# MingXiangL/SPE

Measured on AMD Instinct MI355X. Metric: images/sec (whole node) at 3x800x1333 bs=2/GPU, higher is better.
Workload: dtype bf16/fp16 operands, fp32 accumulate; 1 GPU; TSCAM_cait_S24 (C=384, depth 24, 8 heads) + 0-layer encoder + 6-layer conditional-DETR decoder x2 stages, 100 queries, COCO heads (91), 2x3x800x1333 per GPU (N=4150 tokens), fwd + SetCriterion + SetCriterionRefine + bwd + grad all-reduce + clip + AdamW; global_batch=2, parallelism=dp1

## Files before the change

### include/spe_hip.h

```cpp
#ifndef SPE_HIP_H
#define SPE_HIP_H
#include <stddef.h>
#include <stdint.h>

#ifdef __cplusplus
extern "C" {
#endif

typedef struct ihipStream_t* spe_stream_t;

int spe_abi_version(void);

int spe_set_reduce_workspace(void* ws, size_t bytes, spe_stream_t stream);
int spe_reduce_defer_ranges(const void* const* ptrs, const size_t* bytes, int n);
int spe_reduce_defer_arena(void* arena, size_t bytes);
int spe_reduce_flush(spe_stream_t stream);
int spe_reduce_pending(void);

int spe_gemm_f32(const float* A, const float* B, float* C, const float* bias, float* C2,
                 int M, int N, int K, long lda, long ldb, long ldc, int transA, int transB,
                 int batch0, int batch1, long sA0, long sA1, long sB0, long sB1, long sC0, long sC1,
                 float alpha, int act, int splitk, int precision, spe_stream_t stream);

int spe_gemm_ex(const void* A, int a_bf16, const float* B, float* C, const float* bias, float* C2,
                int M, int N, int K, long lda, long ldb, long ldc, int transA, int transB,
                int batch0, int batch1, long sA0, long sA1, long sB0, long sB1, long sC0, long sC1,
                float alpha, int act, int splitk, int precision, spe_stream_t stream);

int spe_gemm_tile(int M, int N, int nbatch);

int spe_layernorm_fwd(const float* x, const float* gamma, const float* beta, float* y, float* mean,
                      float* rstd, long R, int C, float eps, void* y16, void* y16lo, spe_stream_t stream);
int spe_layernorm_fwd_h(const float* x, const float* gamma, const float* beta, float* y, float* mean,
                        float* rstd, long R, int C, float eps, void* y16, void* yh16, spe_stream_t stream);
int spe_layernorm_bwd(const float* dy, const float* x, const float* gamma, const float* mean,
                      const float* rstd, float* dx, float* dgamma, float* dbeta, long R, int C,
                      const float* add, spe_stream_t stream);
int spe_layernorm_bwd_ls(const float* dy, const float* x, const float* gamma, const float* mean, const float* rstd, float* dx,
                         float* dgamma, float* dbeta, long R, int C, const float* add, const float* ls_y, const float* ls_gamma,
                         void* ls_dy16, float* ls_db, float* ls_dg, spe_stream_t stream);

int spe_cvt_f16(const float* x, long ldx, int R, int C, void* out, long ldo, spe_stream_t stream);
int spe_gemm_bf16nt(const void* A16, const void* B16, const void* A16lo, const void* B16lo, float* C, const float* bias,
                    float* C2, int M, int N, int K, long lda, long ldb, long ldc, float alpha, int act, int splitk,
                    spe_stream_t stream);
int spe_linear_small_fwd(const float* x, long ldx, const void* W16, const void* W16lo, const float* bias, float* y, float* pre,
                         void* x16_out, int R, int N, int K, long ldc, int act, spe_stream_t stream);
int spe_linear_small_bwd(const float* dy, const float* aux, int act, const void* x16, const void* WT16, float* dx, float* dW,
                         float* db, int R, int N, int K, spe_stream_t stream);
int spe_linear_small_group_fwd(const float* x, long ldx, const void* const* W16, const void* const* W16lo, const float* const* bias,
                               const float* const* add, float* const* y, void* x16_out, int R, int nblk, int N, int K, spe_stream_t stream);
int spe_linear_small_group_bwd(const float* const* dy, const void* x16, const void* const* WT16, float* dx, float* const* dW,
                               float* const* db, int R, int nblk, int N, int K, spe_stream_t stream);
int spe_gemm_bf16tn(const void* A16, const void* B16, float* C, int M, int N, int R, long lda, long ldb, long ldc,
                    float alpha, int splitk, spe_stream_t stream);
int spe_gemm_bf16tn_plan(int M, int N, int R, long lda, long ldb, int splitk, int* v);
int spe_gemm_bf16nt_ex(const void* A16, const void* B16, const void* A16lo, const void* B16lo, float* C, const float* bias,
                       float* C2, void* out16, void* out16lo, long ld16, void* out16T, long ld16t, float* colsum, const float* aux,
                       const float* res, const float* rgamma, int M, int N, int K, long lda, long ldb, long ldc, float alpha, int act,
                       int half_flags, spe_stream_t stream);
int spe_gemm_bf16nt_exd(const void* A16, const void* B16, const void* A16lo, const void* B16lo, float* C, const float* bias,
                        float* C2, void* out16, void* out16lo, long ld16, void* out16T, long ld16t, float* colsum, const float* aux,
                        const float* res, const float* rgamma, int M, int N, int K, long lda, long ldb, long ldc, float alpha, int act,
                        int half_flags, float p_drop, uint64_t seed, uint64_t offset, const float* sample_scale, long rows_per_sample,
                        spe_stream_t stream);
int spe_gemm_bf16nt_plan(int M, int N, int K, int split, int ex, int f16_operands, int f16_second, int splitk, int has_out16t,
                         long ld16t, int* plan);
int spe_cvt_bf16(const float* x, long ldx, int R, int C, void* out, void* out_lo, long ldo, void* outT, long ldt, float* colsum,
                 const float* aux, int act, spe_stream_t stream);
int spe_cvt_bf16_h(const float* x, long ldx, int R, int C, void* out, void* out_h, long ldo, void* outT, long ldt, spe_stream_t stream);
int spe_cvt_bf16_multi(const void* jobs_dev, int njobs, int total_tiles, spe_stream_t stream);

int spe_softmax_fwd(const float* S, const unsigned char* mask, float* P, float* Pd, int B, int H, int Nq,
                    int Nk, long ld, float p_drop, uint64_t seed, uint64_t offset, spe_stream_t stream);
int spe_softmax_bwd(const float* dPd, const float* P, float* dS, int B, int H, int Nq, int Nk, long ld,
                    float p_drop, uint64_t seed, uint64_t offset, spe_stream_t stream);

int spe_talking_softmax_fwd(const float* S, const float* Wl, const float* bl, const float* Ww, const float* bw,
                            float* P, float* Pd, int B, int H, int Nq, int Nk, long ld, float p_drop,
                            uint64_t seed, uint64_t offset, spe_stream_t stream);
int spe_talking_softmax_bwd(const float* dPd, const float* P, const float* S, const float* Wl, const float* Ww,
                            float* dS, float* ws, int nblocks, int B, int H, int Nq, int Nk, long ld,
                            float p_drop, uint64_t seed, uint64_t offset, spe_stream_t stream);

int spe_talking_fused_supported(int H, int dh);
int spe_attn_pack(const float* x, long sb, long sn, long sh, int B, int N, int H, int dh, float scale,
                  void* out, spe_stream_t stream);
int spe_talking_stats_plan(int B, int N, int nwg, int* steps_per_wg, int* nwg_used);
int spe_talking_stats(const void* Qf, const void* Kf, const float* Wl, const float* bl, float* ws_stats,
                      int B, int H, int N, int dh, int nwg, spe_stream_t stream);
int spe_attn_merge_rows(const float* ws, float* M, float* IL, const float* bl, float* rows, int Np, int B, int H, int N,
                        int steps_per_wg, spe_stream_t stream);
int spe_talking_wgrad_reduce(const float* ws_w, int nwg, int H, float* dWl, float* dbl, float* dWw, float* dbw,
                             spe_stream_t stream);

int spe_talking_flash_plan(int B, int N, int nwg, int* steps_per_wg, int* nwg_used, int* nmajor, int* rows_padded);
int spe_talking_flash_fwd(const void* Qf, const void* Kf, const void* V16, const float* Wl, const float* Ww, const float* bw,
                          const float* c0, int Np, float* ws, float* O, void* O16, void* O16lo, void* keepbits, int B, int H, int N, int dh,
                          int nwg, float p_drop, uint64_t seed, uint64_t offset, spe_stream_t stream);

int spe_talking_bwdk_pass1(const void* Qf, const void* dOf, const void* dO16, const void* Kf, const void* Vf, const float* Wl, const float* Ww,
                           const float* bw, const float* c0, int Np, float* ws_d, float* ws_v, float* ws_w, float* Drows, float* dv, void* dv16,
                           long ob, long on, long oh, const void* keepbits, int B, int H, int N, int dh, int nwg, float p_drop, spe_stream_t stream);
int spe_talking_bwdq_plan(int B, int N, int nwg, int* steps_per_wg, int* nwg_used, int* nmajor);
int spe_talking_bwdq_pass2(const void* Qf, const void* dOf, const void* Kf, const void* Vf, const void* K16, const float* Wl, const float* Ww,
                           const float* c0, const float* Drows, int Np, float* ws_q, float* ws_w, void* dS, float* dq, void* dq16,
                           long ob, long on, long oh, float scale, const void* keepbits, int B, int H, int N, int dh, int nwg, float p_drop,
                           spe_stream_t stream);

int spe_attn_pmean(const void* Qf, const void* Kf, const float* Wl, const float* c0, int Np, float* M, float alpha, int B, int H, int N, int dh,
                   spe_stream_t stream);
int spe_attn_pmean_dense(const float* P, float* M, float alpha, int B, int H, int N, long ld, spe_stream_t stream);

int spe_conv_head_fwd(const float* x, const float* W, const float* bias, float* map, float* logits, int B, int h, int w, int C, int K,
                      spe_stream_t stream);
int spe_conv_head_plan(int B, int h, int w, int C, int K, long* ws_floats);
int spe_conv_head_bwd(const float* x, const float* W, const float* dmap, const float* dlogits, float* dx, float* dW, float* db, float* ws,
                      long ws_floats, int B, int h, int w, int C, int K, spe_stream_t stream);

int spe_attn_pack16(const float* x, long sb, long sn, long sh, int B, int N, int H, int dh, void* out, spe_stream_t stream);
int spe_attn_pack_multi(int njobs, const float* const* xs, const long* strides, const float* scales, const int* kinds,
                        void* const* outs, const int* Ns, const int* dhs, int B, int H, spe_stream_t stream);
int spe_attn_contract(const void* T, const void* X16, float* out, long ob, long on, long oh, int B, int H, int N, int dh,
                      int trans, int fmt, float alpha, float* ws, unsigned int* counters, long ws_floats, void* out16,
                      void* out16lo, spe_stream_t stream);

int spe_colsum(const float* in, float* out, long R, int C, long ld, int accumulate, spe_stream_t stream);

int spe_layerscale_residual_fwd(const float* x, const float* y, const float* gamma, const float* sample_scale,
                                float* out, long R, int C, long rows_per_sample, spe_stream_t stream);
int spe_layerscale_residual_bwd(const float* dout, const float* y, const float* gamma, const float* sample_scale,
                                float* dy, float* dgamma, long R, int C, long rows_per_sample, spe_stream_t stream);
int spe_layerscale_residual_bwd16(const float* dout, const void* y, int y_f16, const float* gamma, void* dy16, void* dy16T, long ldt,
                                  float* db, float* dgamma, long R, int C, spe_stream_t stream);
int spe_layerscale_residual_bwd16d(const float* dout, const void* y, int y_f16, const float* gamma, void* dy16, void* dy16T, long ldt,
                                   float* db, float* dgamma, long R, int C, float p_drop, uint64_t seed, uint64_t offset,
                                   const float* sample_scale, long rows_per_sample, spe_stream_t stream);

int spe_act_bwd(const float* dy, const float* aux, float* dx, long n, int mode, spe_stream_t stream);

int spe_layernorm_res_fwd(const float* x, const float* z, const float* gamma, const float* beta, float* sum, float* y,
                          float* mean, float* rstd, long R, int C, float eps, float p, uint64_t seed, uint64_t offset,
                          spe_stream_t stream);
int spe_layernorm_res_bwd(const float* dy, const float* dy2, const float* sum, const float* gamma, const float* mean, const float* rstd,
                          float* ds, float* dz, float* dgamma, float* dbeta, long R, int C, float p, uint64_t seed,
                          uint64_t offset, spe_stream_t stream);

int spe_dropout(const float* x, float* y, long n, float p, uint64_t seed, uint64_t offset, spe_stream_t stream);

int spe_patchify(const float* img, float* cols, int B, int Cin, int Hi, int Wi, int P, spe_stream_t stream);

int spe_rowdot(const float* x, const float* y, float* D, int B, int L, int H, int dh, spe_stream_t stream);

int spe_add_rows(const float* a, const float* b, float* out, long n, long period, spe_stream_t stream);

int spe_bicubic(const float* src, float* dst, int gh, int gw, int h, int w, int C, int backward, spe_stream_t stream);

int spe_matcher_cost(const float* logits, const float* boxes, const int* tgt_ids, const float* tgt_boxes,
                     const int* toff, int total_targets, float* cost, int* err, int L, int B, int Q, int Kc,
                     float w_class, float w_bbox, float w_giou, spe_stream_t stream);

int spe_hungarian(const float* cost, const int* toff, long* srow, long* gidx, int* lidx, int* err, int L, int B, int Q,
                  spe_stream_t stream);
int spe_jitter_pick(const float* box, const float* scale, float* out, int M, int ncand, int ratio, spe_stream_t stream);

int spe_focal_loss(const float* logits, const int* tclass, const float* roww, float* grad, float* loss,
                   int* argmax, int L, long rows_per_l, int Kc, float alpha, float gamma, spe_stream_t stream);

int spe_box_loss(const float* pred_boxes, const long* srow, const float* tbox, const float* w, const int* lidx,
                 float* sums, float* g_l1, float* g_giou, long n, int L, spe_stream_t stream);
int spe_box_loss_bwd(const long* srow, const int* lidx, const float* g_l1, const float* g_giou, const float* c1,
                     const float* c2, float* dpred, long n, spe_stream_t stream);

int spe_kv_frags(const void* ym16, long ldm, const void* yp16, long ldp, void* Kf, void* V16, void* K16, void* Vf,
                 int L, int B, int S, int H, int dh, spe_stream_t stream);
int spe_kv_grad_scatter(const float* dk, const float* dv, void* dYm, long ldm, void* dYp, long ldp, int layer, int B, int S,
                        int H, int dh, spe_stream_t stream);
int spe_colsum_bf16_blocks(const void* x, long ld, long R, int nblk, int blkC, float* const* outs, int accumulate, spe_stream_t stream);

int spe_mha_plan(int B, int H, int Lq, int Lk, int* nch);
int spe_mha_fwd(const void* Qf, const void* Kf, const void* V16, const void* mask, float* Opart, float* ML, float* O,
                float* LSE, void* keepbits, int B, int H, int Lq, int Lk, int dk, int dv, int nch, float p_drop,
                uint64_t seed, uint64_t offset, spe_stream_t stream);
int spe_mha_bwd(const void* Qf, const void* Kf, const void* Vf, const void* dOf, const void* K16, const void* Q16,
                const void* dO16, const void* mask, const float* LSE, const float* D, const void* keepbits, float* dq,
                float* dq_ws, float* dk, float* dv, int B, int H, int Lq, int Lk, int dk_dim, int dv_dim, int nch, float scale,
                float p_drop, spe_stream_t stream);

int spe_pos_sine(const void* mask_u8, const float* dim_t, float* out, int B, int h, int w, int npf, float scale,
                 float eps, int normalize, spe_stream_t stream);

int spe_pos_learned_fwd(const float* col, const float* row, float* out, int B, int h, int w, int npf, spe_stream_t stream);
int spe_pos_learned_bwd(const float* g, float* d_col, float* d_row, int B, int h, int w, int npf, spe_stream_t stream);

int spe_nms_sorted(const float* boxes, const long* labels, const int* counts, unsigned char* keep, int nimg, int nmax,
                   float iou_threshold, spe_stream_t stream);

int spe_detect(const float* logits, const float* boxes, const float* sizes, int B, int Q, int Kc, int k, float iou_threshold,
               int do_nms, float* out_logit, long* out_label, float* out_box, int* out_query, int* out_count, spe_stream_t stream);

int spe_cam_prepare(const float* cams, int M, int h, int w, int rows, int cols, float cam_thr, float* minmax,
                    void* out, spe_stream_t stream);
int spe_cam_contour_boxes(const void* img, int rows, int cols, float area_ratio, int* boxes, int max_boxes, int* nboxes);
int spe_cam_boxes_device_workspace(int M, int rows, int cols, size_t* bytes);
int spe_cam_boxes_device(const void* img, int M, int rows, int cols, float area_ratio, void* workspace, size_t workspace_bytes,
                         int* boxes, int* nboxes, int max_boxes, spe_stream_t stream);

int spe_voc_match(const float* det_boxes, const float* det_scores, const long* det_labels, const int* det_off,
                  const double* gt_boxes, const long* gt_labels, const unsigned char* gt_difficult, const int* gt_off,
                  int nimg, int num_classes, int max_det, int max_gt, double ovthresh, double score_scale, double coord_scale,
                  unsigned char* flags, double* scores_out, int* npos, int* nimgs, int* hits, spe_stream_t stream);
int spe_voc_ap(const unsigned char* flags, const int* seg_off, const int* npos, int num_classes, double* ap07, double* ap_area,
               double* rec, double* prec, spe_stream_t stream);

int spe_coco_match(const float* det_boxes, const long* det_cats, const int* det_off, const double* gt_boxes, const long* gt_cats,
                   const unsigned char* gt_iscrowd, const double* gt_area, const int* gt_off, const double* iou_thrs,
                   const double* area_rng, int nimg, int num_cats, int max_det, int max_gt, int top, int* rank, unsigned* words,
                   int* npig, spe_stream_t stream);
int spe_coco_accumulate(const unsigned* words, const int* rank, const float* det_scores, const int* seg_off, const int* npig,
                        const int* max_dets, const double* rec_thrs, int num_cats, int num_rec, int num_max_dets, double* precision,
                        double* recall, double* scores, spe_stream_t stream);

int spe_resample_plan(long* desc_host, int n, long* totals);
int spe_resample_tables(const long* desc_host, const long* desc_dev, int n, int* tables, spe_stream_t stream);
int spe_resample_h(const long* desc_host, const long* desc_dev, int n, const int* tables, unsigned char* tmp, spe_stream_t stream);
int spe_resample_v(const long* desc_host, const long* desc_dev, int n, const int* tables, const unsigned char* tmp, const float* lut,
                   float* out, unsigned char* mask, int Hmax, int Wmax, spe_stream_t stream);

int spe_ledger_state_bytes(int K, int E, size_t* bytes);
int spe_ledger_record(const float* vals, const float* weights, const unsigned char* mask, const double* extras_host, int K, int E,
                      void* state, size_t state_bytes, float* total, spe_stream_t stream);
int spe_ledger_total_bwd(const float* g, const float* weights, const unsigned char* mask, int K, float* dvals, spe_stream_t stream);
int spe_ledger_summary(void* state, size_t state_bytes, int K, int E, const int* windows_host, const int* windows_dev,
                       const float* ring_override, const int* order, double* out, spe_stream_t stream);

int spe_sqnorm_partials(const float* g, long n, float* partials, int nblocks, spe_stream_t stream);
int spe_adamw_flat(float* p, float* g, float* m, float* v, long n, const long* seg_end, const float* seg_lr,
                   const float* seg_wd, int nseg, float beta1, float beta2, float eps, float bias_c1, float bias_c2,
                   const float* partials, int npartials, float max_norm, int write_grad, float grad_scale,
                   spe_stream_t stream);

int spe_accum_flat(float* dst, const float* a, const float* b, long n, spe_stream_t stream);

int spe_occupy(int nwg, long micros, float* buf, long buf_floats, spe_stream_t stream);

#ifdef __cplusplus
}
#endif
#endif
```

### spe_amd/csrc/linear_small.hip

```cpp
#include "common.h"
#include "gemm16_epilogue.h"

#define LS_T 32
#define LS_LDT (LS_T + 8)
#define LS_MAXBLK 16

typedef short s16x4l_t __attribute__((ext_vector_type(4)));
typedef short s16x8l_t __attribute__((ext_vector_type(8)));
typedef __bf16 bf16x4l_t __attribute__((ext_vector_type(4)));

struct LinSmallArgs {
    Gemm16Args g;
    const float* x; long ldx;
    unsigned short* x16;
    const float* aux; int act;
    const unsigned short* xs16;
    float* dW; float* db;
    int R, N, K, tiles_dx;
    int nblk, Nblk;
    const unsigned short* Wb[LS_MAXBLK]; const unsigned short* Wlob[LS_MAXBLK]; const float* biasb[LS_MAXBLK]; float* yb[LS_MAXBLK];
    const float* addb[LS_MAXBLK];
    const float* dyb[LS_MAXBLK]; const unsigned short* WTb[LS_MAXBLK]; float* dWb[LS_MAXBLK]; float* dbb[LS_MAXBLK];
};

__device__ __forceinline__ float ls_dact(float v, float h, int act) {
    if (act == 1) return h > 0.f ? v : 0.f;
    if (act == 2) {
        const float cdf = 0.5f * (1.f + spe_erff(h * 0.70710678118654752f));
        const float pdf = 0.3989422804014327f * __expf(-0.5f * h * h);
        return v * (cdf + h * pdf);
    }
    return v;
}
__device__ __forceinline__ uint2 ls_pack4(float a, float b, float c, float d) {
    bf16x4l_t v; v[0] = (__bf16)a; v[1] = (__bf16)b; v[2] = (__bf16)c; v[3] = (__bf16)d;
    return __builtin_bit_cast(uint2, v);
}

template <int LS_KC, bool SPLIT, bool DACT>
__device__ __forceinline__ void ls_nt_tile(const float* __restrict__ A, long lda, const float* __restrict__ aux, int act, int r0, int R,
                                           const unsigned short* __restrict__ B, const unsigned short* __restrict__ Blo, int n0, int N, int K,
                                           unsigned short* x16, bool write_x16, unsigned short* smem, f32x4_t& acc,
                                           const float* const* Ab = nullptr, const unsigned short* const* Bb = nullptr, int Nblk = 0) {
    constexpr int LS_LD = LS_KC + 8, LS_NA = LS_KC / 32, LS_NB = LS_KC / 64;
    unsigned short* sA = smem;
    unsigned short* sB = sA + LS_T * LS_LD;
    unsigned short* sAl = sB + LS_T * LS_LD;
    unsigned short* sBl = sAl + LS_T * LS_LD;
    const int t = threadIdx.x, lane = t & 63, w = t >> 6, wm = w >> 1, wn = w & 1, fr = lane & 15, fk = (lane >> 4) * 8;
    acc = (f32x4_t){0.f, 0.f, 0.f, 0.f};
    float4 xa[LS_NA], ha[DACT ? LS_NA : 1];
    u32x4g_t wb[LS_NB], wl[SPLIT ? LS_NB : 1];
    auto load = [&](int k0) {
        const int kw = min(LS_KC, K - k0), n4 = kw >> 2, n8 = kw >> 3;
        const float* Ak = A; const unsigned short* Bk = B; long lda_ = lda, ldb_ = K; int kk = k0;
        if (Ab) { const int blk = k0 / Nblk; kk = k0 - blk * Nblk; Ak = Ab[blk]; Bk = Bb[blk]; lda_ = ldb_ = Nblk; }
#pragma unroll
        for (int i = 0; i < LS_NA; ++i) {
            const int rl = (t >> 5) + 8 * (i & 3), c4 = (t & 31) + 32 * (i >> 2);
            if (c4 >= n4) continue;
            const long off = (long)min(r0 + rl, R - 1) * lda_ + kk + c4 * 4;
            xa[i] = Ak ? *reinterpret_cast<const float4*>(Ak + off) : make_float4(0.f, 0.f, 0.f, 0.f);
            if constexpr (DACT) { if (aux) ha[i] = *reinterpret_cast<const float4*>(aux + off); }
        }
#pragma unroll
        for (int i = 0; i < LS_NB; ++i) {
            const int nl = (t >> 4) + 16 * (i & 1), c8 = (t & 15) + 16 * (i >> 1);
            if (c8 >= n8) continue;
            const long off = (long)min(n0 + nl, N - 1) * ldb_ + kk + c8 * 8;
            wb[i] = *reinterpret_cast<const u32x4g_t*>(Bk + off);
            if constexpr (SPLIT) wl[i] = *reinterpret_cast<const u32x4g_t*>(Blo + off);
        }
    };
    load(0);
    for (int k0 = 0; k0 < K; k0 += LS_KC) {
        const int kw = min(LS_KC, K - k0), n4 = kw >> 2, n8 = kw >> 3;
        const int kpad = (kw + 31) & ~31;
#pragma unroll
        for (int i = 0; i < LS_NA; ++i) {
            const int rl = (t >> 5) + 8 * (i & 3), c4 = (t & 31) + 32 * (i >> 2);
            if (c4 >= n4) continue;
            float4 v = xa[i];
            if (r0 + rl >= R) v = make_float4(0.f, 0.f, 0.f, 0.f);
            if constexpr (DACT) {
                if (aux) { v.x = ls_dact(v.x, ha[i].x, act); v.y = ls_dact(v.y, ha[i].y, act); v.z = ls_dact(v.z, ha[i].z, act); v.w = ls_dact(v.w, ha[i].w, act); }
            }
            bf16x4l_t h; h[0] = (__bf16)v.x; h[1] = (__bf16)v.y; h[2] = (__bf16)v.z; h[3] = (__bf16)v.w;
            const uint2 uh = __builtin_bit_cast(uint2, h);
            *reinterpret_cast<uint2*>(sA + rl * LS_LD + c4 * 4) = uh;
            if constexpr (SPLIT) *reinterpret_cast<uint2*>(sAl + rl * LS_LD + c4 * 4) = ls_pack4(v.x - (float)h[0], v.y - (float)h[1], v.z - (float)h[2], v.w - (float)h[3]);
            if (write_x16 && r0 + rl < R) *reinterpret_cast<uint2*>(x16 + (long)(r0 + rl) * K + k0 + c4 * 4) = uh;
        }
#pragma unroll
        for (int i = 0; i < LS_NB; ++i) {
            const int nl = (t >> 4) + 16 * (i & 1), c8 = (t & 15) + 16 * (i >> 1);
            if (c8 >= n8) continue;
            const bool nv = n0 + nl < N;
            *reinterpret_cast<u32x4g_t*>(sB + nl * LS_LD + c8 * 8) = nv ? wb[i] : (u32x4g_t){0u, 0u, 0u, 0u};
            if constexpr (SPLIT) *reinterpret_cast<u32x4g_t*>(sBl + nl * LS_LD + c8 * 8) = nv ? wl[i] : (u32x4g_t){0u, 0u, 0u, 0u};
        }
        if (kpad > kw && t < 2 * LS_T * ((kpad - kw) >> 3)) {
            const int per = (kpad - kw) >> 3, idx = t % (LS_T * per), rl = idx / per, c8 = idx % per;
            unsigned short* base = (t < LS_T * per) ? sA : sB;
            *reinterpret_cast<u32x4g_t*>(base + rl * LS_LD + kw + c8 * 8) = (u32x4g_t){0u, 0u, 0u, 0u};
            if constexpr (SPLIT) *reinterpret_cast<u32x4g_t*>((base == sA ? sAl : sBl) + rl * LS_LD + kw + c8 * 8) = (u32x4g_t){0u, 0u, 0u, 0u};
        }
        if (k0 + LS_KC < K) load(k0 + LS_KC);
        __syncthreads();
        const int arow = (wm * 16 + fr) * LS_LD + fk, brow = (wn * 16 + fr) * LS_LD + fk;
        for (int ks = 0; ks < kpad; ks += 32) {
            const bf16x8_t a = __builtin_bit_cast(bf16x8_t, *reinterpret_cast<const u16x8_t*>(sA + arow + ks));
            const bf16x8_t b = __builtin_bit_cast(bf16x8_t, *reinterpret_cast<const u16x8_t*>(sB + brow + ks));
            if constexpr (SPLIT) {
                const bf16x8_t al = __builtin_bit_cast(bf16x8_t, *reinterpret_cast<const u16x8_t*>(sAl + arow + ks));
                const bf16x8_t bl = __builtin_bit_cast(bf16x8_t, *reinterpret_cast<const u16x8_t*>(sBl + brow + ks));
                acc = __builtin_amdgcn_mfma_f32_16x16x32_bf16(bl, a, acc, 0, 0, 0);
                acc = __builtin_amdgcn_mfma_f32_16x16x32_bf16(b, al, acc, 0, 0, 0);
            }
            acc = __builtin_amdgcn_mfma_f32_16x16x32_bf16(b, a, acc, 0, 0, 0);
        }
        if (k0 + LS_KC < K) __syncthreads();
    }
}

template <int KC, bool SPLIT>
__global__ __launch_bounds__(256) void linear_small_fwd_kernel(LinSmallArgs p) {
    extern __shared__ __attribute__((aligned(16))) unsigned short ls_smem[];
    const int tiles_r = (p.g.M + LS_T - 1) / LS_T;
    const int tr = blockIdx.x % tiles_r, tn = blockIdx.x / tiles_r;
    f32x4_t acc1;
    if (p.nblk > 0) {
        const int blk = tn * LS_T / p.Nblk, tl = tn - blk * (p.Nblk / LS_T);
        ls_nt_tile<KC, SPLIT, false>(p.x, p.ldx, nullptr, 0, tr * LS_T, p.g.M, p.Wb[blk], p.Wlob[blk], tl * LS_T, p.Nblk, p.g.K, p.x16,
                                 p.x16 != nullptr && tn == 0, ls_smem, acc1);
        Gemm16Args g = p.g;
        g.C = p.yb[blk]; g.bias = p.biasb[blk]; g.N = p.Nblk; g.ldc = p.Nblk;
        if (p.addb[blk]) {
            const int lane = threadIdx.x & 63, w = threadIdx.x >> 6;
            const int m = tr * LS_T + (w >> 1) * 16 + (lane & 15), n = tl * LS_T + (w & 1) * 16 + (lane >> 4) * 4;
            if (m < p.g.M && n + 3 < p.Nblk) {
                const float4 a4 = *reinterpret_cast<const float4*>(p.addb[blk] + (long)m * p.Nblk + n);
                acc1[0] += a4.x; acc1[1] += a4.y; acc1[2] += a4.z; acc1[3] += a4.w;
            }
        }
        f32x4_t accg[1][1] = {{acc1}};
        gemm16_epilogue_plain<LS_T, LS_T>(g, accg, g.C, tr * LS_T, tl * LS_T);
        return;
    }
    ls_nt_tile<KC, SPLIT, false>(p.x, p.ldx, nullptr, 0, tr * LS_T, p.g.M, p.g.B, p.g.Blo, tn * LS_T, p.g.N, p.g.K, p.x16, p.x16 != nullptr && tn == 0,
                             ls_smem, acc1);
    f32x4_t acc[1][1] = {{acc1}};
    gemm16_epilogue_plain<LS_T, LS_T>(p.g, acc, p.g.C, tr * LS_T, tn * LS_T);
}

__device__ __forceinline__ bf16x8_t ls_operand_t(const unsigned short* tile, int ks, int c0, int lane) {
    typedef __attribute__((address_space(3))) s16x4l_t lds_s4;
    const unsigned short* q = tile + (32 * ks + 8 * (lane >> 4) + ((lane & 15) >> 2)) * LS_LDT + c0 + 4 * (lane & 3);
    const s16x4l_t v0 = __builtin_amdgcn_ds_read_tr16_b64_v4i16((lds_s4*)(q));
    const s16x4l_t v1 = __builtin_amdgcn_ds_read_tr16_b64_v4i16((lds_s4*)(q + 4 * LS_LDT));
    const s16x8l_t v = __builtin_shufflevector(v0, v1, 0, 1, 2, 3, 4, 5, 6, 7);
    return __builtin_bit_cast(bf16x8_t, v);
}

template <int KC, int LS_RC>
__global__ __launch_bounds__(256) void linear_small_bwd_kernel(LinSmallArgs p) {
    constexpr int LS_ND = LS_RC / 32, LS_NX = LS_RC / 64;
    extern __shared__ __attribute__((aligned(16))) unsigned short ls_smem[];
    const int R = p.R, N = p.N, K = p.K;
    const int t = threadIdx.x, lane = t & 63, w = t >> 6, wm = w >> 1, wn = w & 1, fr = lane & 15;
    if ((int)blockIdx.x < p.tiles_dx) {
        const int tiles_r = (R + LS_T - 1) / LS_T;
        const int tr = blockIdx.x % tiles_r, tk = blockIdx.x / tiles_r;
        f32x4_t acc1;
        if (p.nblk > 0) ls_nt_tile<KC, false, true>(nullptr, 0, nullptr, 0, tr * LS_T, R, nullptr, nullptr, tk * LS_T, K, N, nullptr, false, ls_smem, acc1,
                                                    p.dyb, p.WTb, p.Nblk);
        else ls_nt_tile<KC, false, true>(p.x, N, p.aux, p.act, tr * LS_T, R, p.g.B, nullptr, tk * LS_T, K, N, nullptr, false, ls_smem, acc1);
        const int r = tr * LS_T + wm * 16 + fr, k = tk * LS_T + wn * 16 + (lane >> 4) * 4;
        if (r < R && k < K) *reinterpret_cast<float4*>(p.g.C + (long)r * K + k) = make_float4(acc1[0], acc1[1], acc1[2], acc1[3]);
        return;
    }
    unsigned short* sD = ls_smem;
    unsigned short* sX = sD + LS_RC * LS_LDT;
    float* sred = reinterpret_cast<float*>(sX + LS_RC * LS_LDT);
    const int b2 = blockIdx.x - p.tiles_dx;
    const int tiles_n = (N + LS_T - 1) / LS_T;
    const int tn = b2 % tiles_n, tk = b2 / tiles_n;
    int n0 = tn * LS_T; const int k0 = tk * LS_T;
    const float* dyp = p.x; float* dWp = p.dW; float* dbp = p.db; int Nld = N;
    if (p.nblk > 0) {
        const int blk = n0 / p.Nblk;
        n0 -= blk * p.Nblk; Nld = p.Nblk;
        dyp = p.dyb[blk]; dWp = p.dWb[blk]; dbp = p.dbb[blk];
        if (!dyp) return;
    }
    const bool want_dw = dWp != nullptr, want_db = dbp != nullptr && tk == 0;
    f32x4_t acc = {0.f, 0.f, 0.f, 0.f};
    float4 bsum = make_float4(0.f, 0.f, 0.f, 0.f);
    float4 dv[LS_ND], hv[LS_ND]; u32x4g_t xv[LS_NX];
    auto load = [&](int rc0) {
        const int cn = n0 + (t & 7) * 4, ck = k0 + (t & 3) * 8;
#pragma unroll
        for (int i = 0; i < LS_ND; ++i) {
            const int r = rc0 + (t >> 3) + 32 * i;
            if (r >= R) continue;
            const long off = (long)min(r, R - 1) * Nld + min(cn, Nld - 4);
            dv[i] = *reinterpret_cast<const float4*>(dyp + off);
            if (p.aux) hv[i] = *reinterpret_cast<const float4*>(p.aux + off);
        }
        if (want_dw) {
#pragma unroll
            for (int i = 0; i < LS_NX; ++i) {
                const int r = rc0 + (t >> 2) + 64 * i;
                if (r >= R) continue;
                xv[i] = *reinterpret_cast<const u32x4g_t*>(p.xs16 + (long)min(r, R - 1) * K + min(ck, K - 8));
            }
        }
    };
    load(0);
    for (int rc0 = 0; rc0 < R; rc0 += LS_RC) {
        const int rows = min(LS_RC, R - rc0), rpad = (rows + 31) & ~31;
        const bool cnv = n0 + (t & 7) * 4 < Nld, ckv = k0 + (t & 3) * 8 < K;
#pragma unroll
        for (int i = 0; i < LS_ND; ++i) {
            const int rl = (t >> 3) + 32 * i;
            if (rl >= rpad) continue;
            float4 v = dv[i];
            if (p.aux) { v.x = ls_dact(v.x, hv[i].x, p.act); v.y = ls_dact(v.y, hv[i].y, p.act); v.z = ls_dact(v.z, hv[i].z, p.act); v.w = ls_dact(v.w, hv[i].w, p.act); }
            if (rl >= rows || !cnv) v = make_float4(0.f, 0.f, 0.f, 0.f);
            bsum.x += v.x; bsum.y += v.y; bsum.z += v.z; bsum.w += v.w;
            *reinterpret_cast<uint2*>(sD + rl * LS_LDT + (t & 7) * 4) = ls_pack4(v.x, v.y, v.z, v.w);
        }
        if (want_dw) {
#pragma unroll
            for (int i = 0; i < LS_NX; ++i) {
                const int rl = (t >> 2) + 64 * i;
                if (rl >= rpad) continue;
                *reinterpret_cast<u32x4g_t*>(sX + rl * LS_LDT + (t & 3) * 8) = (rl < rows && ckv) ? xv[i] : (u32x4g_t){0u, 0u, 0u, 0u};
            }
        }
        if (rc0 + LS_RC < R) load(rc0 + LS_RC);
        __syncthreads();
        if (want_dw) {
            for (int ks = 0; ks < rpad / 32; ++ks) {
                const bf16x8_t a = ls_operand_t(sD, ks, wm * 16, lane);
                const bf16x8_t b = ls_operand_t(sX, ks, wn * 16, lane);
                acc = __builtin_amdgcn_mfma_f32_16x16x32_bf16(b, a, acc, 0, 0, 0);
            }
        }
        if (rc0 + LS_RC < R) __syncthreads();
    }
    if (want_dw) {
        const int n = n0 + wm * 16 + fr, k = k0 + wn * 16 + (lane >> 4) * 4;
        if (n < Nld && k < K) *reinterpret_cast<float4*>(dWp + (long)n * K + k) = make_float4(acc[0], acc[1], acc[2], acc[3]);
    }
    if (want_db) {
        __syncthreads();
        *reinterpret_cast<float4*>(sred + (t >> 3) * 32 + (t & 7) * 4) = bsum;
        __syncthreads();
        if (t < LS_T && n0 + t < Nld) {
            float s = 0.f;
#pragma unroll
            for (int i = 0; i < 32; ++i) s += sred[i * 32 + t];
            dbp[n0 + t] = s;
        }
    }
}

static int ls_latency_tiles() {
    static int v = -1;
    if (v < 0) v = SPE_KNOB("SPE_LS_WIDE_MAX", 320);
    return v;
}

extern "C" int spe_linear_small_fwd(const float* x, long ldx, const void* W16, const void* W16lo, const float* bias, float* y, float* pre,
                                    void* x16_out, int R, int N, int K, long ldc, int act, hipStream_t stream) {
    if (R <= 0 || N <= 0) return 0;
    auto al16 = [](const void* q) { return (reinterpret_cast<uintptr_t>(q) & 15) == 0; };
    if (K <= 0 || (K & 7) || (ldx & 3) || !al16(x) || !al16(W16) || !al16(W16lo) || !al16(x16_out)) return -2;
    LinSmallArgs p = {};
    p.g.B = reinterpret_cast<const unsigned short*>(W16); p.g.Blo = reinterpret_cast<const unsigned short*>(W16lo);
    p.g.C = y; p.g.C2 = pre; p.g.bias = bias; p.g.M = R; p.g.N = N; p.g.K = K; p.g.ldc = ldc; p.g.alpha = 1.f; p.g.act = act; p.g.splitk = 1;
    p.x = x; p.ldx = ldx; p.x16 = reinterpret_cast<unsigned short*>(x16_out);
    const int tiles = ((R + LS_T - 1) / LS_T) * ((N + LS_T - 1) / LS_T);
    const bool split = W16lo != nullptr;
    const bool wide = tiles <= ls_latency_tiles();
    const int smem = (split ? 4 : 2) * LS_T * ((wide ? 384 : 128) + 8) * (int)sizeof(unsigned short);
    static bool attr_set = false;
    if (!attr_set) {
        hipError_t e = hipFuncSetAttribute(reinterpret_cast<const void*>(&linear_small_fwd_kernel<384, true>), hipFuncAttributeMaxDynamicSharedMemorySize,
                                           4 * LS_T * 392 * (int)sizeof(unsigned short));
        if (e != hipSuccess) return (int)e;
        attr_set = true;
    }
    if (wide) {
        if (split) hipLaunchKernelGGL((linear_small_fwd_kernel<384, true>), dim3(tiles), dim3(256), smem, stream, p);
        else hipLaunchKernelGGL((linear_small_fwd_kernel<384, false>), dim3(tiles), dim3(256), smem, stream, p);
    } else {
        if (split) hipLaunchKernelGGL((linear_small_fwd_kernel<128, true>), dim3(tiles), dim3(256), smem, stream, p);
        else hipLaunchKernelGGL((linear_small_fwd_kernel<128, false>), dim3(tiles), dim3(256), smem, stream, p);
    }
    SPE_CHECK_LAUNCH();
    return 0;
}

extern "C" int spe_linear_small_bwd(const float* dy, const float* aux, int act, const void* x16, const void* WT16, float* dx, float* dW,
                                    float* db, int R, int N, int K, hipStream_t stream) {
    if (R <= 0 || N <= 0 || K <= 0) return 0;
    auto al16 = [](const void* q) { return (reinterpret_cast<uintptr_t>(q) & 15) == 0; };
    if ((K & 7) || (N & 7) || !al16(dy) || !al16(aux) || !al16(x16) || !al16(WT16) || !al16(dx) || !al16(dW)) return -2;
    if ((dx && !WT16) || (dW && !x16) || (aux && act != 1 && act != 2)) return -2;
    LinSmallArgs p = {};
    p.x = dy; p.aux = aux; p.act = act; p.xs16 = reinterpret_cast<const unsigned short*>(x16);
    p.g.B = reinterpret_cast<const unsigned short*>(WT16); p.g.C = dx;
    p.dW = dW; p.db = db; p.R = R; p.N = N; p.K = K;
    const int tr = (R + LS_T - 1) / LS_T, tk = (K + LS_T - 1) / LS_T, tn = (N + LS_T - 1) / LS_T;
    p.tiles_dx = dx ? tr * tk : 0;
    const int tiles_dw = dW ? tn * tk : (db ? tn : 0);
    if (p.tiles_dx + tiles_dw == 0) return 0;
    const bool wide = p.tiles_dx + tiles_dw <= ls_latency_tiles();
    auto smem_of = [](int kc, int rc) { const int a = 2 * LS_T * (kc + 8) * 2, b = 2 * rc * LS_LDT * 2 + 32 * 32 * 4; return a > b ? a : b; };
    static bool attr_set = false;
    if (!attr_set) {
        hipError_t e = hipFuncSetAttribute(reinterpret_cast<const void*>(&linear_small_bwd_kernel<384, 512>), hipFuncAttributeMaxDynamicSharedMemorySize,
                                           smem_of(384, 512));
        if (e != hipSuccess) return (int)e;
        attr_set = true;
    }
    if (wide) hipLaunchKernelGGL((linear_small_bwd_kernel<384, 512>), dim3(p.tiles_dx + tiles_dw), dim3(256), smem_of(384, 512), stream, p);
    else hipLaunchKernelGGL((linear_small_bwd_kernel<128, 256>), dim3(p.tiles_dx + tiles_dw), dim3(256), smem_of(128, 256), stream, p);
    SPE_CHECK_LAUNCH();
    return 0;
}

static bool ls_group_kc_wide(int N) { return N % 384 == 0; }
extern "C" int spe_linear_small_group_fwd(const float* x, long ldx, const void* const* W16, const void* const* W16lo, const float* const* bias,
                                          const float* const* add, float* const* y, void* x16_out, int R, int nblk, int N, int K, hipStream_t stream) {
    if (R <= 0 || N <= 0 || nblk <= 0) return 0;
    auto al16 = [](const void* q) { return (reinterpret_cast<uintptr_t>(q) & 15) == 0; };
    if (nblk > LS_MAXBLK || K <= 0 || (K & 7) || (N % LS_T) || (ldx & 3) || !al16(x) || !al16(x16_out)) return -2;
    LinSmallArgs p = {};
    const bool split = W16lo != nullptr;
    for (int i = 0; i < nblk; ++i) {
        if (!W16[i] || !y[i] || !al16(W16[i]) || !al16(y[i]) || (split && (!W16lo[i] || !al16(W16lo[i])))) return -2;
        p.Wb[i] = reinterpret_cast<const unsigned short*>(W16[i]); p.Wlob[i] = split ? reinterpret_cast<const unsigned short*>(W16lo[i]) : nullptr;
        p.biasb[i] = bias ? bias[i] : nullptr; p.yb[i] = y[i];
        p.addb[i] = add ? add[i] : nullptr;
        if (p.addb[i] && (!al16(p.addb[i]) || (N & 3))) return -2;
    }
    p.nblk = nblk; p.Nblk = N;
    p.g.M = R; p.g.N = nblk * N; p.g.K = K; p.g.ldc = N; p.g.alpha = 1.f; p.g.act = 0; p.g.splitk = 1;
    p.x = x; p.ldx = ldx; p.x16 = reinterpret_cast<unsigned short*>(x16_out);
    const int tiles = ((R + LS_T - 1) / LS_T) * (nblk * N / LS_T);
    const bool wide = tiles <= ls_latency_tiles();
    const int smem = (split ? 4 : 2) * LS_T * ((wide ? 384 : 128) + 8) * (int)sizeof(unsigned short);
    static bool attr_set = false;
    if (!attr_set) {
        hipError_t e = hipFuncSetAttribute(reinterpret_cast<const void*>(&linear_small_fwd_kernel<384, true>), hipFuncAttributeMaxDynamicSharedMemorySize,
                                           4 * LS_T * 392 * (int)sizeof(unsigned short));
        if (e != hipSuccess) return (int)e;
        attr_set = true;
    }
    if (wide) {
        if (split) hipLaunchKernelGGL((linear_small_fwd_kernel<384, true>), dim3(tiles), dim3(256), smem, stream, p);
        else hipLaunchKernelGGL((linear_small_fwd_kernel<384, false>), dim3(tiles), dim3(256), smem, stream, p);
    } else {
        if (split) hipLaunchKernelGGL((linear_small_fwd_kernel<128, true>), dim3(tiles), dim3(256), smem, stream, p);
        else hipLaunchKernelGGL((linear_small_fwd_kernel<128, false>), dim3(tiles), dim3(256), smem, stream, p);
    }
    SPE_CHECK_LAUNCH();
    return 0;
}

extern "C" int spe_linear_small_group_bwd(const float* const* dy, const void* x16, const void* const* WT16, float* dx, float* const* dW,
                                          float* const* db, int R, int nblk, int N, int K, hipStream_t stream) {
    if (R <= 0 || N <= 0 || K <= 0 || nblk <= 0) return 0;
    auto al16 = [](const void* q) { return (reinterpret_cast<uintptr_t>(q) & 15) == 0; };
    if (nblk > LS_MAXBLK || (K & 7) || (N % 128) || !al16(x16) || !al16(dx) || (dx && !WT16) || (dW && !x16)) return -2;
    LinSmallArgs p = {};
    bool any_dw = false;
    for (int i = 0; i < nblk; ++i) {
        p.dyb[i] = dy[i]; p.WTb[i] = WT16 ? reinterpret_cast<const unsigned short*>(WT16[i]) : nullptr;
        p.dWb[i] = dW ? dW[i] : nullptr; p.dbb[i] = db ? db[i] : nullptr;
        if (!al16(p.dyb[i]) || !al16(p.WTb[i]) || !al16(p.dWb[i]) || (dx && !p.WTb[i])) return -2;
        any_dw = any_dw || (p.dyb[i] && (p.dWb[i] || p.dbb[i]));
    }
    p.nblk = nblk; p.Nblk = N;
    p.xs16 = reinterpret_cast<const unsigned short*>(x16); p.g.C = dx;
    p.R = R; p.N = nblk * N; p.K = K;
    const int tr = (R + LS_T - 1) / LS_T, tk = (K + LS_T - 1) / LS_T, tn = nblk * N / LS_T;
    p.tiles_dx = dx ? tr * tk : 0;
    const int tiles_dw = any_dw ? tn * tk : 0;
    if (p.tiles_dx + tiles_dw == 0) return 0;
    const bool wide = ls_group_kc_wide(N) && p.tiles_dx + tiles_dw <= ls_latency_tiles();
    auto smem_of = [](int kc, int rc) { const int a = 2 * LS_T * (kc + 8) * 2, b = 2 * rc * LS_LDT * 2 + 32 * 32 * 4; return a > b ? a : b; };
    static bool attr_set = false;
    if (!attr_set) {
        hipError_t e = hipFuncSetAttribute(reinterpret_cast<const void*>(&linear_small_bwd_kernel<384, 512>), hipFuncAttributeMaxDynamicSharedMemorySize,
                                           smem_of(384, 512));
        if (e != hipSuccess) return (int)e;
        attr_set = true;
    }
    if (wide) hipLaunchKernelGGL((linear_small_bwd_kernel<384, 512>), dim3(p.tiles_dx + tiles_dw), dim3(256), smem_of(384, 512), stream, p);
    else hipLaunchKernelGGL((linear_small_bwd_kernel<128, 256>), dim3(p.tiles_dx + tiles_dw), dim3(256), smem_of(128, 256), stream, p);
    SPE_CHECK_LAUNCH();
    return 0;
}
```

### spe_amd/kernels.py

```python
import ctypes
import os

import torch

from . import lib

_PRECISION = 2
import functools as _functools
import threading as _threading

_TLS = _threading.local()


def _in_bwd():
    return getattr(_TLS, "in_bwd", False)


def backward_scope(fn):
    @_functools.wraps(fn)
    def wrapped(ctx, *grads):
        prev, _TLS.in_bwd = _in_bwd(), True
        if _DEFER_FLATS is not None and not _FLUSH_QUEUED[0]:
            _FLUSH_QUEUED[0] = True
            try:
# ... 419 lines not shown
    _WCATH[key] = ([weakref.ref(W._base if W._base is not None else W) for W in Ws], _W16_EPOCH, vers, Wh, bc)
    return Wh, bc


def kv_frags(ym16, yp16, L, B, S, H, dh, train):
    dev = ym16.device
    nt, dk = (S + 15) // 16, 2 * dh
    Kf = torch.empty((L, B, H, nt, (dk + 31) // 32, 64, 8), device=dev, dtype=torch.float16)
    V16 = torch.empty((L, B, H, nt, (dh + 15) // 16, 64, 4), device=dev, dtype=torch.float16)
    K16 = torch.empty((L, B, H, nt, (dk + 15) // 16, 64, 4), device=dev, dtype=torch.bfloat16) if train else None
    Vf = torch.empty((L, B, H, nt, (dh + 31) // 32, 64, 8), device=dev, dtype=torch.bfloat16) if train else None
    _call("spe_kv_frags", _p(ym16), ym16.stride(0), _p(yp16), yp16.stride(0), _p(Kf), _p(V16), _p(K16), _p(Vf), L, B, S, H, dh, _st())
    return Kf, V16, K16, Vf


def kv_grad_scatter(dk, dv, dYm, dYp, layer, B, S, H, dh):
    _call("spe_kv_grad_scatter", _p(dk), _p(dv), _p(dYm), dYm.stride(0), _p(dYp), dYp.stride(0), int(layer), B, S, H, dh, _st())


def colsum_bf16_blocks(x16, blkC, outs):
    n = len(outs)
    ptrs = (ctypes.c_void_p * n)(*[o.data_ptr() for o in outs])
    _call("spe_colsum_bf16_blocks", _p(x16), x16.stride(0), x16.shape[0], n, int(blkC), ptrs, 0, _st())


def gemm16_tn(A16, B16, C, M, N, R, lda, ldb, ldc, alpha=1.0, splitk=1):
    _call("spe_gemm_bf16tn", _p(A16), _p(B16), _p(C), M, N, R, lda, ldb, ldc, float(alpha), int(splitk), _st())
    return C


def gemm16_tn_plan(M, N, R, splitk=1, lda=None, ldb=None):
    v = (ctypes.c_int * 4)()
    rc = lib.load().spe_gemm_bf16tn_plan(M, N, R, M if lda is None else lda, N if ldb is None else ldb, int(splitk), v)
    if rc != 0:
        return None
    return dict(BM=v[0], BN=v[1], splits=v[2], rt_per_split=v[3])


def gemm16_ex(A16, B16, M, N, K, lda, ldb, bias=None, C=None, C2=None, out16=None, out16T=None, colsum=None, aux=None,
              alpha=1.0, act=0, res=None, rgamma=None, Alo=None, Blo=None, out16lo=None, drop=None, sscale=None, rps=1, op_f16=False):
    half_flags = (1 if (C2 is not None and C2.dtype == torch.float16) else 0) | (2 if (aux is not None and aux.dtype == torch.float16) else 0)
    if op_f16:
        assert A16.dtype == torch.float16 and B16.dtype == torch.float16 and Alo is None and Blo is None
        half_flags |= 4 | (8 if out16lo is not None else 0)
        assert out16lo is None or out16lo.dtype == torch.float16
    if (drop is not None and drop[0] > 0) or sscale is not None:
        pd, sd, of = drop if (drop is not None and drop[0] > 0) else (0.0, 0, 0)
        _call("spe_gemm_bf16nt_exd", _p(A16), _p(B16), _p(Alo), _p(Blo), _p(C), _p(bias), _p(C2), _p(out16), _p(out16lo), N, _p(out16T),
              out16T.shape[1] if out16T is not None else 0, _p(colsum), _p(aux), _p(res), _p(rgamma), M, N, K, lda, ldb, N,
              float(alpha), int(act), half_flags, float(pd), int(sd), int(of), _p(sscale), int(rps), _st())
        return
    _call("spe_gemm_bf16nt_ex", _p(A16), _p(B16), _p(Alo), _p(Blo), _p(C), _p(bias), _p(C2), _p(out16), _p(out16lo), N, _p(out16T),
          out16T.shape[1] if out16T is not None else 0, _p(colsum), _p(aux), _p(res), _p(rgamma), M, N, K, lda, ldb, N,
          float(alpha), int(act), half_flags, _st())


def mlp16_ok(R, K, Hd, N):
    return _lin16_ok(R, Hd, K) and _lin16_ok(R, N, Hd)




def layerscale_residual_bwd16(dout2, y2, gamma, Rp, db_out=None, dg_out=None, want_rowmajor=True, want_T=True, drop=None, sscale=None, rps=1):
    R, C = dout2.shape
    dev = dout2.device
    dy16 = torch.empty((R, C), device=dev, dtype=torch.bfloat16) if want_rowmajor else None
    dy16T = torch.empty((C, Rp), device=dev, dtype=torch.bfloat16) if want_T else None
    db = _zeros_or(db_out, C, dev)
    dg = _zeros_or(dg_out, C, dev)
    if (drop is not None and drop[0] > 0) or sscale is not None:
        pd, sd, of = drop if (drop is not None and drop[0] > 0) else (0.0, 0, 0)
        _call("spe_layerscale_residual_bwd16d", _p(dout2), _p(y2), int(y2.dtype == torch.float16), _p(gamma), _p(dy16), _p(dy16T), Rp, _p(db),
              _p(dg), R, C, float(pd), int(sd), int(of), _p(sscale), int(rps), _st())
        return dy16, dy16T, db, dg
    _call("spe_layerscale_residual_bwd16", _p(dout2), _p(y2), int(y2.dtype == torch.float16), _p(gamma), _p(dy16), _p(dy16T), Rp, _p(db), _p(dg),
          R, C, _st())
    return dy16, dy16T, db, dg


def linear_res_fwd(x2, W, b, res, gamma, save=True, src=None, drop=None, sscale=None, rps=1):
    R, K = x2.shape
    N = W.shape[0]
    dev = x2.device
    sp = split_fwd()
    x16, x16lo = act16(x2, src, want_lo=sp)
    out = torch.empty((R, N), device=dev, dtype=torch.float32)
    y = torch.empty((R, N), device=dev, dtype=torch.float16 if MLP_PRE_F16 else torch.float32) if save else None
    Wt = weight16(W, lo=sp)
    gemm16_ex(x16, Wt[0], R, N, K, K, K, bias=b, C=out, C2=y, res=res, rgamma=gamma, Alo=x16lo, Blo=Wt[2] if sp else None,
              drop=drop, sscale=sscale, rps=rps)
    return out, (x16, y)


def linear_res_bwd(dout2, saved, W, gamma, need_dx=True, grad_bufs=(None, None, None), drop=None, sscale=None, rps=1, pre=None):
    x16, y = saved
    R, N = dout2.shape
    K = W.shape[1]
    gW, gb, gg = grad_bufs
    if pre is not None:
        dy16, db, dg = pre
    else:
        dy16, _, db, dg = layerscale_residual_bwd16(dout2, y, gamma, ((R + 63) // 64) * 64, db_out=gb, dg_out=gg, want_rowmajor=True, want_T=False,
                                                    drop=drop, sscale=sscale, rps=rps)
    dW = _dw16_tn(dy16, x16, N, K, R, gW)
    dx = None
    if need_dx:
        dx = torch.empty((R, K), device=dout2.device, dtype=torch.float32)
        gemm16(dy16, weight16(W)[1], dx, R, K, N, N, N, K)
    return dx, dW, db, dg


MLP_PRE_F16 = False


MLP_F16 = True


def gemm16_plan(M, N, K, split=False, ex=False, op_f16=False, lo_f16=False, splitk=1, out16T=False, ld16t=0):
    v = (ctypes.c_int * 9)()
    rc = lib.load().spe_gemm_bf16nt_plan(M, N, K, int(split), int(ex), int(op_f16), int(lo_f16), int(splitk), int(out16T), int(ld16t), v)
    if rc != 0:
        return None
    return dict(family=("nt2", "bf16nt")[v[0]], BM=v[1], BN=v[2], BK=v[3], NST=v[4], NTS=v[5], SPLIT=bool(v[6]), EX=bool(v[7]), F16=bool(v[8]))


def mlp_f16_ok(R, K, Hd, N):
    return (MLP_F16 and split_fwd() and R >= 2048 and K % 64 == 0 and K >= 128 and Hd % 64 == 0 and Hd >= 128 and N % 8 == 0 and N >= 64)


def mlp_gelu_fwd(x2, W1, b1, W2, b2, res=None, gamma=None, save=True, src=None, drop1=None, drop2=None, sscale=None, rps=1):
    R, K = x2.shape
    Hd, N = W1.shape[0], W2.shape[0]
    dev = x2.device
    sp = split_fwd()
    if res is not None and mlp_f16_ok(R, K, Hd, N):
        x16, xh = act16(x2, src, want_lo=True, lo_f16=True)
        pre = torch.empty((R, Hd), device=dev, dtype=torch.float16 if MLP_PRE_F16 else torch.float32) if save else None
        h16 = torch.empty((R, Hd), device=dev, dtype=torch.bfloat16)
        hh = torch.empty((R, Hd), device=dev, dtype=torch.float16)
        W1h, W2h = weight16(W1, lo=True, f16=True)[2], weight16(W2, lo=True, f16=True)[2]
        gemm16_ex(xh, W1h, R, Hd, K, K, K, bias=b1, C2=pre, out16=h16, act=2, out16lo=hh, drop=drop1, op_f16=True)
        out = torch.empty((R, N), device=dev, dtype=torch.float32)
        y = torch.empty((R, N), device=dev, dtype=torch.float16 if MLP_PRE_F16 else torch.float32) if save else None
        gemm16_ex(hh, W2h, R, N, Hd, Hd, Hd, bias=b2, C=out, C2=y, res=res, rgamma=gamma, drop=drop2, sscale=sscale, rps=rps, op_f16=True)
        return out, (x16, pre, h16, y)
    x16, x16lo = act16(x2, src, want_lo=sp)
    pre = torch.empty((R, Hd), device=dev, dtype=torch.float16 if MLP_PRE_F16 else torch.float32) if save else None
    h16 = torch.empty((R, Hd), device=dev, dtype=torch.bfloat16)
    h16lo = torch.empty((R, Hd), device=dev, dtype=torch.bfloat16) if sp else None
    W1t, W2t = weight16(W1, lo=sp), weight16(W2, lo=sp)
    W1lo, W2lo = (W1t[2], W2t[2]) if sp else (None, None)
    gemm16_ex(x16, W1t[0], R, Hd, K, K, K, bias=b1, C2=pre, out16=h16, act=2, Alo=x16lo, Blo=W1lo, out16lo=h16lo, drop=drop1)
    y = torch.empty((R, N), device=dev, dtype=torch.float32)
    if res is None:
        gemm16(h16, W2t[0], y, R, N, Hd, Hd, Hd, N, bias=b2, Alo=h16lo, Blo=W2lo)
        return y, (x16, pre, h16)
    out = torch.empty((R, N), device=dev, dtype=torch.float32)
    if MLP_PRE_F16:
        y = torch.empty((R, N), device=dev, dtype=torch.float16)
    gemm16_ex(h16, W2t[0], R, N, Hd, Hd, Hd, bias=b2, C=out, C2=y if save else None, res=res, rgamma=gamma, Alo=h16lo, Blo=W2lo,
              drop=drop2, sscale=sscale, rps=rps)
    return out, (x16, pre, h16, y)


def _dw_slabs(launch, sk, N, K, dW_out, dev):
    if sk > 1:
        ws = torch.empty((sk, N * K), device=dev, dtype=torch.float32)
        launch(ws, -sk)
        return colsum(ws, out=None if dW_out is None else dW_out.view(-1), accumulate=dW_out is None).view(N, K)
    dW = dW_out if dW_out is not None else torch.empty((N, K), device=dev, dtype=torch.float32)
    launch(dW, 1)
    return dW


def _dw16_tn(dy16, x16, N, K, R, dW_out, lda=None):
    lda = N if lda is None else lda
    sk = min(auto_splitk(N, K, R, 1), max(1, R // 64))
    return _dw_slabs(lambda C, splitk: gemm16_tn(dy16, x16, C, N, K, R, lda, K, K, splitk=splitk), sk, N, K, dW_out, dy16.device)


def mlp_gelu_bwd(dy2, saved, W1, W2, need_dx=True, grad_bufs=(None, None, None, None), gamma=None, dg_out=None,
                 drop1=None, drop2=None, sscale=None, rps=1, ls_pre=None):
    x16, pre, h16 = saved[:3]
    R, N = dy2.shape
    Hd, K = W1.shape
    dev = dy2.device
    gW1, gb1, gW2, gb2 = grad_bufs
    dg = None
    if ls_pre is not None and gamma is None:
        raise RuntimeError("spe_amd.kernels.mlp_gelu_bwd: a LayerNorm backward took this node's LayerScale part, but the node cannot consume it")
    if ls_pre is not None:
        dy16, db2, dg = ls_pre
    elif gamma is not None:
        dy16, _, db2, dg = layerscale_residual_bwd16(dy2, saved[3], gamma, ((R + 63) // 64) * 64, db_out=gb2, dg_out=dg_out, want_T=False,
                                                     drop=drop2, sscale=sscale, rps=rps)
    else:
        db2 = _zeros_or(gb2, N, dev)
        dy16, _ = cvt_bf16(dy2, True, False, colsum_out=db2)
    dW2 = _dw16_tn(dy16, h16, N, Hd, R, gW2)
    db1 = _zeros_or(gb1, Hd, dev)
    dp16 = torch.empty((R, Hd), device=dev, dtype=torch.bfloat16)
    gemm16_ex(dy16, weight16(W2)[1], R, Hd, N, N, N, out16=dp16, colsum=db1, aux=pre, act=2, drop=drop1)
    dW1 = _dw16_tn(dp16, x16, Hd, K, R, gW1)
    dx = None
    if need_dx:
        dx = torch.empty((R, K), device=dev, dtype=torch.float32)
        gemm16(dp16, weight16(W1)[1], dx, R, K, Hd, Hd, Hd, K)
    if gamma is not None:
        return dx, dW1, db1, dW2, db2, dg
    return dx, dW1, db1, dW2, db2


def act16(x2, src=None, want_lo=False, lo_f16=False):
    if src is not None:
        ent = getattr(src, "_spe16", None)
        if (ent is not None and ent[0] == src._version and ent[1].shape == x2.shape
                and (not want_lo or (ent[3] is not None and (ent[3].dtype == torch.float16) == lo_f16))):
            return ent[1], (ent[3] if want_lo else None)
    x16lo = torch.empty(x2.shape, device=x2.device, dtype=torch.float16 if lo_f16 else torch.bfloat16) if want_lo else None
    x16, _ = cvt_bf16(x2, True, False, out_lo=x16lo, lo_f16=lo_f16 and want_lo)
    if src is not None:
        attach16(src, x16, x16lo)
    return x16, x16lo


def linear_fwd(x2, W, b, act=0, want_pre=False, save_for_dw=True, src=None):
    _chk(x2, W, b)
    R, K = x2.shape
    N = W.shape[0]
    y = torch.empty((R, N), device=x2.device, dtype=torch.float32)
    pre = torch.empty_like(y) if want_pre else None
    if _lin_small_ok(R, N, K) and W.is_contiguous():
        sp = split_fwd()
        Wt = weight16(W, lo=sp)
        ent = getattr(src, "_spe16", None) if src is not None else None
        x16 = ent[1] if (ent is not None and ent[0] == src._version and ent[1].shape == x2.shape) else None
        x16_out = None
        if x16 is None and save_for_dw:
            x16 = x16_out = torch.empty((R, K), device=x2.device, dtype=torch.bfloat16)
            if src is not None:
                attach16(src, x16)
        _call("spe_linear_small_fwd", _p(x2), x2.stride(0), _p(Wt[0]), _p(Wt[2] if sp else None), _p(b), _p(y), _p(pre), _p(x16_out),
              R, N, K, N, int(act), _st())
        return y, pre, (x16 if save_for_dw else x2)
    if _lin16_ok(R, N, K) and W.is_contiguous():
        sp = split_fwd()
        x16, x16lo = act16(x2, src, want_lo=sp)
        Wt = weight16(W, lo=sp)
        gemm16(x16, Wt[0], y, R, N, K, K, K, N, bias=b, C2=pre, act=act, Alo=x16lo, Blo=Wt[2] if sp else None)
        return y, pre, (x16 if save_for_dw else x2)
    gemm(x2, W, y, R, N, K, K, K, N, False, True, bias=b, C2=pre, act=act)
    return y, pre, x2


def linear_group_ok(R, Ws, bs):
    N, K = Ws[0].shape
    return (2 <= len(Ws) <= 16 and _lin_small_ok(R, N, K) and N % 128 == 0
            and all(W.shape == Ws[0].shape and W.is_contiguous() for W in Ws) and all(b is not None for b in bs))


def _ptr_array(ptrs):
    return (ctypes.c_void_p * len(ptrs))(*[(p if p else None) for p in ptrs])


def linear_group_fwd(x2, Ws, bs, src=None, adds=None):
    _chk(x2, *Ws)
    R, K = x2.shape
    N = Ws[0].shape[0]
    sp = split_fwd()
    trip = [weight16(W, lo=sp) for W in Ws]
    ent = getattr(src, "_spe16", None) if src is not None else None
    x16 = ent[1] if (ent is not None and ent[0] == src._version and ent[1].shape == x2.shape) else None
    x16_out = None
    if x16 is None:
        x16 = x16_out = torch.empty((R, K), device=x2.device, dtype=torch.bfloat16)
        if src is not None:
            attach16(src, x16)
    ys = [torch.empty((R, N), device=x2.device, dtype=torch.float32) for _ in Ws]
    _call("spe_linear_small_group_fwd", _p(x2), x2.stride(0), _ptr_array([t_[0].data_ptr() for t_ in trip]),
          _ptr_array([t_[2].data_ptr() for t_ in trip]) if sp else None, _ptr_array([b.data_ptr() for b in bs]),
          _ptr_array([0 if a is None else a.data_ptr() for a in adds]) if adds is not None else None,
          _ptr_array([y.data_ptr() for y in ys]), _p(x16_out), R, len(Ws), N, K, _st())
    return ys, x16


def linear_group_bwd(dys, x16, Ws, need_dx, dW_outs, db_outs):
    n = len(Ws)
    N, K = Ws[0].shape
    R = x16.shape[0]
    dev = x16.device
    dx = torch.empty((R, K), device=dev, dtype=torch.float32) if need_dx else None
    dWs, dbs = [], []
    for i in range(n):
        if dys[i] is None:
            dWs.append(None); dbs.append(None)
            continue
        dWs.append(dW_outs[i] if dW_outs[i] is not None else torch.empty((N, K), device=dev, dtype=torch.float32))
        dbs.append(db_outs[i].view(-1) if db_outs[i] is not None else torch.empty((N,), device=dev, dtype=torch.float32))
    _call("spe_linear_small_group_bwd", _ptr_array([0 if d is None else d.data_ptr() for d in dys]), _p(x16),
          _ptr_array([weight16(W)[1].data_ptr() for W in Ws]) if need_dx else None, _p(dx),
          _ptr_array([0 if w is None else w.data_ptr() for w in dWs]), _ptr_array([0 if b is None else b.data_ptr() for b in dbs]),
          R, n, N, K, _st())
    return dx, dWs, dbs


def linear_bwd(dy2, xsave, W, need_dx=True, need_dw=True, need_db=True, dW_out=None, db_out=None, act=0, act_aux=None):
    _chk(dy2, W)
    R, N = dy2.shape
    K = W.shape[1]
    dx = dW = db = None
    x16 = xsave.dtype == torch.bfloat16
    if (x16 or not need_dw) and _lin_small_ok(R, N, K) and W.is_contiguous():
        dev = dy2.device
        if need_dx:
            dx = torch.empty((R, K), device=dev, dtype=torch.float32)
        if need_dw:
            dW = dW_out if dW_out is not None else torch.empty((N, K), device=dev, dtype=torch.float32)
        if need_db:
            db = db_out.view(-1) if db_out is not None else torch.empty((N,), device=dev, dtype=torch.float32)
        _call("spe_linear_small_bwd", _p(dy2), _p(act_aux if act else None), int(act), _p(xsave if need_dw else None),
              _p(weight16(W)[1] if need_dx else None), _p(dx), _p(dW), _p(db), R, N, K, _st())
        return dx, dW, db
    if (x16 or not need_dw) and _lin16_ok(R, N, K) and W.is_contiguous():
        if need_db:
            db = _zeros_or(db_out, N, dy2.device)
        dy16, _ = cvt_bf16(dy2, need_dx or need_dw, False, colsum_out=db, act_aux=act_aux if act else None, act=act)
        need_db = False
        if need_dx:
            dx = torch.empty((R, K), device=dy2.device, dtype=torch.float32)
            gemm16(dy16, weight16(W)[1], dx, R, K, N, N, N, K)
        if need_dw:
            dW = _dw16_tn(dy16, xsave, N, K, R, dW_out)
    else:
        if x16:
            raise RuntimeError("linear_bwd: bf16 activations were saved but the bf16 GEMM path is disabled now")
        if act:
            dy2 = act_bwd(dy2, act_aux, act)
        x2 = xsave
        if need_dx:
            dx = torch.empty((R, K), device=dy2.device, dtype=torch.float32)
            gemm(dy2, W, dx, R, K, N, N, K, K, False, False)
        if need_dw:
            dW = _dw_slabs(lambda C, splitk: gemm(dy2, x2, C, N, K, R, N, K, K, True, False, splitk=splitk), auto_splitk(N, K, R, 1), N, K,
                           dW_out, dy2.device)
    if need_db:
        db = _zeros_or(db_out, N, dy2.device)
        _call("spe_colsum", _p(dy2), _p(db), R, N, N, 1, _st())
    return dx, dW, db


def colsum(x2, out=None, accumulate=True):
    _chk(x2)
    R, C = x2.shape
    if out is None:
        out = zeros_small(C, x2.device)
    _call("spe_colsum", _p(x2), _p(out), R, C, x2.stride(0), int(bool(accumulate)), _st())
    return out


def act_bwd(dy, aux, mode):
    _chk(dy, aux)
    dx = torch.empty_like(dy)
    _call("spe_act_bwd", _p(dy), _p(aux), _p(dx), dy.numel(), mode, _st())
    return dx


def layernorm_fwd(x2, g, b, eps, want16=False, f16=False):
    _chk(x2, g, b)
    R, C = x2.shape
    y = torch.empty_like(x2)
    mean = torch.empty((R,), device=x2.device, dtype=torch.float32)
    rstd = torch.empty_like(mean)
    y16 = torch.empty((R, C), device=x2.device, dtype=torch.bfloat16) if want16 else None
    f16 = f16 and want16 and split_fwd()
    y16lo = torch.empty((R, C), device=x2.device, dtype=torch.float16 if f16 else torch.bfloat16) if (want16 and split_fwd()) else None
    _call("spe_layernorm_fwd_h" if f16 else "spe_layernorm_fwd", _p(x2), _p(g), _p(b), _p(y), _p(mean), _p(rstd), R, C, float(eps), _p(y16), _p(y16lo), _st())
    return (y, mean, rstd, y16, y16lo) if want16 else (y, mean, rstd)


def produces16(R, C):
    return LINEAR16 and _PRECISION != 1 and R >= LINEAR16_MIN_ROWS and C % 8 == 0


def attach16(t, x16, x16lo=None):
    t._spe16 = (t._version, x16, None, x16lo)


LN_LS_FUSE = True


def layernorm_bwd(dy2, x2, g, mean, rstd, dg_out=None, db_out=None, add=None, ls=None):
    _chk(dy2, x2, g)
    R, C = x2.shape
    dx = torch.empty_like(x2)
    dg = _zeros_or(dg_out, C, x2.device)
    db = _zeros_or(db_out, C, x2.device)
    if ls is not None:
        y, lgam, ls_db_out, ls_dg_out = ls
        dy16 = torch.empty((R, C), device=x2.device, dtype=torch.bfloat16)
        ldb = _zeros_or(ls_db_out, C, x2.device)
        ldg = _zeros_or(ls_dg_out, C, x2.device)
        _call("spe_layernorm_bwd_ls", _p(dy2), _p(x2), _p(g), _p(mean), _p(rstd), _p(dx), _p(dg), _p(db), R, C, _p(add), _p(y), _p(lgam), _p(dy16),
              _p(ldb), _p(ldg), _st())
        return dx, dg, db, (dy16, ldb, ldg)
    _call("spe_layernorm_bwd", _p(dy2), _p(x2), _p(g), _p(mean), _p(rstd), _p(dx), _p(dg), _p(db), R, C, _p(add), _st())
    return dx, dg, db


def layernorm_res_fwd(x2, z2, g, b, eps, p, seed, offset):
    _chk(x2, z2, g, b)
    R, C = x2.shape
    y, sm = torch.empty_like(x2), torch.empty_like(x2)
    mean = torch.empty((R,), device=x2.device, dtype=torch.float32)
    rstd = torch.empty_like(mean)
    _call("spe_layernorm_res_fwd", _p(x2), _p(z2), _p(g), _p(b), _p(sm), _p(y), _p(mean), _p(rstd), R, C, float(eps), float(p), seed,
          offset, _st())
    return y, sm, mean, rstd


def layernorm_res_bwd(dy2, sm, g, mean, rstd, p, seed, offset, dg_out=None, db_out=None, dy_b=None):
    R, C = sm.shape
    ds = torch.empty_like(sm)
    dz = torch.empty_like(sm) if p > 0 else None
    dg = _zeros_or(dg_out, C, sm.device)
    db = _zeros_or(db_out, C, sm.device)
    _call("spe_layernorm_res_bwd", _p(dy2), _p(dy_b), _p(sm), _p(g), _p(mean), _p(rstd), _p(ds), _p(dz), _p(dg), _p(db), R, C, float(p), seed,
          offset, _st())
    return ds, (dz if dz is not None else ds), dg, db


def layerscale_residual_fwd(x2, y2, gamma, sample_scale, rows_per_sample):
    _chk(x2, y2, gamma, sample_scale)
    R, C = x2.shape
    out = torch.empty_like(x2)
    _call("spe_layerscale_residual_fwd", _p(x2), _p(y2), _p(gamma), _p(sample_scale), _p(out), R, C,
             rows_per_sample, _st())
    return out


def layerscale_residual_bwd(dout2, y2, gamma, sample_scale, rows_per_sample, dg_out=None):
    _chk(dout2, y2, gamma, sample_scale)
    R, C = dout2.shape
    dy = torch.empty_like(dout2)
    dg = _zeros_or(dg_out, C, dout2.device)
    _call("spe_layerscale_residual_bwd", _p(dout2), _p(y2), _p(gamma), _p(sample_scale), _p(dy), _p(dg), R, C,
             rows_per_sample, _st())
    return dy, dg


def dropout(x, p, seed, offset):
    _chk(x)
    y = torch.empty_like(x)
    _call("spe_dropout", _p(x), _p(y), x.numel(), float(p), seed, offset, _st())
    return y


def pad4(n):
    return (n + 3) // 4 * 4


def softmax_fwd(S, mask_u8, B, H, Nq, Nk, ld, p_drop, seed, offset):
    Pd = torch.empty_like(S) if p_drop > 0 else None
    _call("spe_softmax_fwd", _p(S), _p(mask_u8), _p(S), _p(Pd), B, H, Nq, Nk, ld, float(p_drop), seed, offset, _st())
    return S, Pd


def softmax_bwd(dPd, P, B, H, Nq, Nk, ld, p_drop, seed, offset):
    _call("spe_softmax_bwd", _p(dPd), _p(P), _p(dPd), B, H, Nq, Nk, ld, float(p_drop), seed, offset, _st())
    return dPd


def talking_fwd(S, Wl, bl, Ww, bw, B, H, Nq, Nk, ld, p_drop, seed, offset):
    Pd = torch.empty_like(S)
    _call("spe_talking_softmax_fwd", _p(S), _p(Wl), _p(bl), _p(Ww), _p(bw), _p(S), _p(Pd), B, H, Nq, Nk, ld,
             float(p_drop), seed, offset, _st())
    return S, Pd


def talking_bwd(dPd, P, S, Wl, Ww, B, H, Nq, Nk, ld, p_drop, seed, offset):
    nblocks = min(B * Nq, 1024)
    nw = 2 * (H * H + H)
    ws = torch.empty((nblocks, nw), device=dPd.device, dtype=torch.float32)
    _call("spe_talking_softmax_bwd", _p(dPd), _p(P), _p(S), _p(Wl), _p(Ww), _p(dPd), _p(ws), nblocks, B, H, Nq, Nk, ld,
             float(p_drop), seed, offset, _st())
    g = colsum(ws)
    hh = H * H
    return dPd, g[:hh].view(H, H), g[hh:hh + H], g[hh + H:2 * hh + H].view(H, H), g[2 * hh + H:]


def patchify(img, P):
    _chk(img)
    B, Cin, Hi, Wi = img.shape
    h, w = Hi // P, Wi // P
    cols = torch.empty((B * h * w, Cin * P * P), device=img.device, dtype=torch.float32)
    _call("spe_patchify", _p(img), _p(cols), B, Cin, Hi, Wi, P, _st())
    return cols


def add_rows(a, table):
    _chk(a, table)
    out = torch.empty_like(a)
    _call("spe_add_rows", _p(a), _p(table), _p(out), a.numel(), table.numel(), _st())
    return out


def matcher_cost(logits, boxes, tgt_ids_i32, tgt_boxes, toff_i32, total_targets, w_class, w_bbox, w_giou):
    _chk(logits, boxes, tgt_boxes)
    L, B, Q, Kc = logits.shape
    cost = torch.empty((L, Q * total_targets), device=logits.device, dtype=torch.float32)
    err = torch.zeros((1,), device=logits.device, dtype=torch.int32)
    _call("spe_matcher_cost", _p(logits), _p(boxes), _p(tgt_ids_i32), _p(tgt_boxes), _p(toff_i32), total_targets,
             _p(cost), _p(err), L, B, Q, Kc, float(w_class), float(w_bbox), float(w_giou), _st())
    return cost, err


def hungarian(cost, toff_i32, L, B, Q, total_targets, err=None):
    dev = cost.device
    srow = torch.empty((L * total_targets,), device=dev, dtype=torch.int64)
    gidx = torch.empty_like(srow)
    lidx = torch.empty((L * total_targets,), device=dev, dtype=torch.int32)
    _call("spe_hungarian", _p(cost), _p(toff_i32), _p(srow), _p(gidx), _p(lidx), _p(err), L, B, Q, _st())
    return srow, gidx, lidx


def focal_loss(logits, tclass_i32, roww, alpha, gamma):
    _chk(logits, roww)
    L, R, Kc = logits.shape
    grad = torch.empty_like(logits)
    loss = torch.zeros((L,), device=logits.device, dtype=torch.float32)
    amax = torch.empty((L, R), device=logits.device, dtype=torch.int32)
    _call("spe_focal_loss", _p(logits), _p(tclass_i32), _p(roww), _p(grad), _p(loss), _p(amax), L, R, Kc,
             float(alpha), float(gamma), _st())
    return loss, grad, amax


def box_loss(pred_boxes, srow_i64, tbox, w, lidx_i32, L):
    _chk(pred_boxes, tbox, w)
    n = srow_i64.numel()
    sums = torch.zeros((L, 2), device=pred_boxes.device, dtype=torch.float32)
    g1 = torch.empty((n, 4), device=pred_boxes.device, dtype=torch.float32)
    g2 = torch.empty_like(g1)
    _call("spe_box_loss", _p(pred_boxes), _p(srow_i64), _p(tbox), _p(w), _p(lidx_i32), _p(sums), _p(g1), _p(g2), n, int(L), _st())
    return sums, g1, g2


def box_loss_bwd(srow_i64, lidx_i32, g1, g2, c1, c2, shape):
    dpred = torch.zeros(shape, device=g1.device, dtype=torch.float32)
    _call("spe_box_loss_bwd", _p(srow_i64), _p(lidx_i32), _p(g1), _p(g2), _p(c1), _p(c2), _p(dpred), srow_i64.numel(), _st())
    return dpred


STATS_NWG = 512
_STATS_NWG_SOLO = STATS_NWG


def set_cu_reserve(n):
    global _CU_RESERVE, STATS_NWG
    _CU_RESERVE = int(n)
    STATS_NWG = max(8, (_STATS_NWG_SOLO - int(n)) & ~7) if n > 0 else _STATS_NWG_SOLO


_CU_RESERVE = 0


def get_cu_reserve():
    return _CU_RESERVE


@_functools.lru_cache(maxsize=None)
def fused_supported(H, dh):
    return bool(lib.load().spe_talking_fused_supported(H, dh))


LOG2E = 1.4426950408889634


def attn_pack(x4, scale=1.0):
    _chk(x4)
    B, N, H, dh = x4.shape
    nt = (N + 15) // 16
    out = torch.empty((B, H, nt, frag_record_elems(dh)), device=x4.device, dtype=torch.bfloat16)
    _call("spe_attn_pack", _p(x4), x4.stride(0), x4.stride(1), x4.stride(2), B, N, H, dh, float(scale), _p(out), _st())
    return out


_PLANS = {}


def fused_plan(B, N):
    key = ("stats", B, N, STATS_NWG)
    r = _PLANS.get(key)
    if r is None:
        spw, nwg = ctypes.c_int(0), ctypes.c_int(0)
        lib.call("spe_talking_stats_plan", B, N, STATS_NWG, ctypes.byref(spw), ctypes.byref(nwg))
        r = _PLANS[key] = (spw.value, nwg.value)
    return r


STATS_SLOTS = 8


def talking_stats(Qf, Kf, Wl, bl, ws_stats, B, H, N, dh):
    _call("spe_talking_stats", _p(Qf), _p(Kf), _p(Wl), _p(bl), _p(ws_stats), B, H, N, dh, STATS_NWG, _st())


def score_blocks(B, H, N, device, dtype=torch.bfloat16):
    nt = (N + 15) // 16
    return torch.empty((B, H, nt, nt, 64, 4), device=device, dtype=dtype)


def attn_pack16(x4):
    B, N, H, dh = x4.shape
    assert x4.stride(3) == 1
    nt, DT = (N + 15) // 16, (dh + 15) // 16
    out = torch.empty((B, H, nt, DT, 64, 4), device=x4.device, dtype=torch.bfloat16)
    _call("spe_attn_pack16", _p(x4), x4.stride(0), x4.stride(1), x4.stride(2), B, N, H, dh, _p(out), _st())
    return out


def frag_record_elems(dh):
    rem = dh % 32
    full = dh // 32 + (1 if rem > 16 else 0)
    return full * 512 + (256 if 0 < rem <= 16 else 0)


F16 = 1000


def attn_pack_multi(jobs):
    B, _, H, _ = jobs[0][0].shape
    n = len(jobs)
    outs = []
    for x4, scale, kind in jobs:
        Bn, N, Hn, dh = x4.shape
        assert Bn == B and Hn == H and x4.stride(3) == 1 and x4.dtype == torch.float32
        nt = (N + 15) // 16
        if kind % F16 == 32:
            shape = (B, H, nt, frag_record_elems(dh))
        elif kind % F16 == 322:
            shape = (B, H, nt, (dh + 31) // 32, 64, 8)
        else:
            shape = (B, H, nt, (dh + 15) // 16, 64, 4)
        outs.append(torch.empty(shape, device=x4.device, dtype=torch.float16 if kind >= F16 else torch.bfloat16))
    xs = (ctypes.c_void_p * n)(*[j[0].data_ptr() for j in jobs])
    strides = (ctypes.c_long * (3 * n))(*[s for j in jobs for s in (j[0].stride(0), j[0].stride(1), j[0].stride(2))])
    scales = (ctypes.c_float * n)(*[float(j[1]) for j in jobs])
    kinds = (ctypes.c_int * n)(*[{32: 0, 16: 1, 322: 2}[j[2] % F16] + (16 if j[2] >= F16 else 0) for j in jobs])
    optr = (ctypes.c_void_p * n)(*[o.data_ptr() for o in outs])
    Ns = (ctypes.c_int * n)(*[j[0].shape[1] for j in jobs])
    dhs = (ctypes.c_int * n)(*[j[0].shape[3] for j in jobs])
    _call("spe_attn_pack_multi", n, xs, strides, scales, kinds, optr, Ns, dhs, B, H, _st())
    return outs

# ... 554 lines not shown
```

### spe_amd/models/transformer.py

```python
import copy
import math

import torch
from torch import nn

from .. import ops
from .attention import MultiheadAttention
from .layers import MLP, Dropout, LayerNorm, Linear


def gen_sineembed_for_position(pos_tensor, d_model=256):
    n_steps = d_model // 2
    scale = 2 * math.pi
    dim_t = torch.arange(n_steps, dtype=torch.float32, device=pos_tensor.device)
    dim_t = 10000 ** (2 * torch.div(dim_t, 2, rounding_mode="floor") / 128)
    pos_x = pos_tensor[..., 0, None] * scale / dim_t
    pos_y = pos_tensor[..., 1, None] * scale / dim_t
    pos_x = torch.stack((pos_x[..., 0::2].sin(), pos_x[..., 1::2].cos()), dim=-1).flatten(-2)
    pos_y = torch.stack((pos_y[..., 0::2].sin(), pos_y[..., 1::2].cos()), dim=-1).flatten(-2)
    return torch.cat((pos_y, pos_x), dim=-1)


class PackedSelfAttention(nn.Module):

    def __init__(self, embed_dim, num_heads, dropout=0.0):
        super().__init__()
        self.embed_dim, self.num_heads, self.dropout = embed_dim, num_heads, float(dropout)
        self.in_proj_weight = nn.Parameter(torch.empty(3 * embed_dim, embed_dim))
        self.in_proj_bias = nn.Parameter(torch.zeros(3 * embed_dim))
        self.out_proj = Linear(embed_dim, embed_dim)
        nn.init.xavier_uniform_(self.in_proj_weight)
        nn.init.constant_(self.out_proj.bias, 0.0)

    def forward(self, qk_in, v_in, key_padding_mask):
        B, S, d = qk_in.shape
        H = self.num_heads
        qk = ops.linear(qk_in, self.in_proj_weight[:2 * d], self.in_proj_bias[:2 * d]).view(B, S, 2, H, d // H)
        v = ops.linear(v_in, self.in_proj_weight[2 * d:], self.in_proj_bias[2 * d:]).view(B, S, H, d // H)
        o, _ = ops.attention(qk[:, :, 0], qk[:, :, 1], v, key_padding_mask, float(d // H) ** -0.5,
                             self.dropout if self.training else 0.0)
        return self.out_proj(o)


class TransformerEncoderLayer(nn.Module):
    def __init__(self, d_model, nhead, dim_feedforward=2048, dropout=0.1, activation="relu", normalize_before=False):
        super().__init__()
        if normalize_before:
            raise NotImplementedError("pre-norm is not reachable in the reference (transformer.py:461-462)")
        self.self_attn = PackedSelfAttention(d_model, nhead, dropout=dropout)
        self.linear1 = Linear(d_model, dim_feedforward)
        self.dropout = Dropout(dropout)
        self.linear2 = Linear(dim_feedforward, d_model)
        self.norm1 = LayerNorm(d_model)
        self.norm2 = LayerNorm(d_model)
        self.dropout1 = Dropout(dropout)
        self.dropout2 = Dropout(dropout)

    def forward(self, src, src_key_padding_mask=None, pos=None):
        qk = src if pos is None else ops.add(src, pos)
        src2 = self.self_attn(qk, src, src_key_padding_mask)
        src, src_skip = self.norm1.residual2(src, src2, self.dropout1)
        src2 = self.linear2(self.dropout(self.linear1(src, ops.ACT_RELU)))
        return self.norm2.residual(src_skip, src2, self.dropout2)


class TransformerEncoder(nn.Module):
    def __init__(self, encoder_layer, num_layers, norm=None):
        super().__init__()
        self.layers = _get_clones(encoder_layer if num_layers != 0 else nn.Identity(), max(num_layers, 1))
        self.num_layers = num_layers
        self.norm = norm

    def forward(self, src, src_key_padding_mask=None, pos=None):
        out = src
        if self.num_layers:
            for layer in self.layers:
                out = layer(out, src_key_padding_mask=src_key_padding_mask, pos=pos)
        return out if self.norm is None else self.norm(out)


class TransformerDecoderLayer(nn.Module):
    def __init__(self, d_model, nhead, dim_feedforward=2048, dropout=0.1, activation="relu", normalize_before=False):
        super().__init__()
        self.sa_qcontent_proj = Linear(d_model, d_model)
        self.sa_qpos_proj = Linear(d_model, d_model)
        self.sa_kcontent_proj = Linear(d_model, d_model)
        self.sa_kpos_proj = Linear(d_model, d_model)
        self.sa_v_proj = Linear(d_model, d_model)
        self.self_attn = MultiheadAttention(d_model, nhead, dropout=dropout, vdim=d_model)
        self.ca_qcontent_proj = Linear(d_model, d_model)
        self.ca_qpos_proj = Linear(d_model, d_model)
        self.ca_kcontent_proj = Linear(d_model, d_model)
        self.ca_kpos_proj = Linear(d_model, d_model)
        self.ca_v_proj = Linear(d_model, d_model)
        self.ca_qpos_sine_proj = Linear(d_model, d_model)
        self.cross_attn = MultiheadAttention(d_model * 2, nhead, dropout=dropout, vdim=d_model)
        self.nhead = nhead
        self.linear1 = Linear(d_model, dim_feedforward)
        self.dropout = Dropout(dropout)
        self.linear2 = Linear(dim_feedforward, d_model)
        self.norm1 = LayerNorm(d_model)
        self.norm2 = LayerNorm(d_model)
        self.norm3 = LayerNorm(d_model)
        self.dropout1 = Dropout(dropout)
        self.dropout2 = Dropout(dropout)
        self.dropout3 = Dropout(dropout)

    def memory_side(self, memory, pos, is_first):
        B, S, d = memory.shape
        H, dh = self.nhead, d // self.nhead
        k_content = self.ca_kcontent_proj(memory)
        v = self.ca_v_proj(memory)
        k_pos = self.ca_kpos_proj(pos)
        k = ops.add(k_content, k_pos) if is_first else k_content
        k = torch.cat([k.view(B, S, H, dh), k_pos.view(B, S, H, dh)], dim=3)
        return k.view(B, S, 2 * d), v

    def forward(self, tgt, mem_kv, memory_key_padding_mask, query_pos, query_sine_embed, is_first, n_stages=1, qp=None):
        B, RQ, d = tgt.shape
        H, dh = self.nhead, d // self.nhead
        Q = RQ // n_stages
        q_pos, k_pos, ca_pos = qp if qp is not None else (self.sa_qpos_proj(query_pos), self.sa_kpos_proj(query_pos), None)
        content = (self.sa_qcontent_proj, self.sa_kcontent_proj, self.sa_v_proj)
        if ops.group_linear_ok(tgt, content):
            q, k, v = ops.group_linear(tgt, content, adds=(q_pos, k_pos, None))
        else:
            q, k, v = (m(tgt) for m in content)
            q = q + q_pos
            k = k + k_pos
        sa = lambda t: t.view(B * n_stages, Q, d)
        tgt2 = self.self_attn(sa(q), sa(k), sa(v))[0].view(B, RQ, d)
        tgt, tgt_skip = self.norm1.residual2(tgt, tgt2, self.dropout1)
        q = self.ca_qcontent_proj(tgt)
        if is_first:
            q = q + (ca_pos if ca_pos is not None else self.ca_qpos_proj(query_pos))
        qs = self.ca_qpos_sine_proj(query_sine_embed)
        if isinstance(mem_kv[0], ops.MemoryKV):
            holder, tok, layer_id = mem_kv
            if is_first:
                qs = qs + q
            q = torch.cat([q.view(B, RQ, H, dh), qs.view(B, RQ, H, dh)], dim=3)
            ca = self.cross_attn
            o = ops.cross_attention_kv(q, tok, holder, layer_id, memory_key_padding_mask, float(ca.head_dim) ** -0.5,
                                       ca.dropout if ca.training else 0.0)
            tgt2 = ca.out_proj(o)
        else:
            q = torch.cat([q.view(B, RQ, H, dh), qs.view(B, RQ, H, dh)], dim=3).view(B, RQ, 2 * d)
            k, v = mem_kv
            tgt2 = self.cross_attn(q, k, v, key_padding_mask=memory_key_padding_mask)[0]
        tgt, tgt_skip = self.norm2.residual2(tgt_skip, tgt2, self.dropout2)
        tgt2 = self.linear2(self.dropout(self.linear1(tgt, ops.ACT_RELU)))
        return self.norm3.residual(tgt_skip, tgt2, self.dropout3)


class TransformerDecoder(nn.Module):
    def __init__(self, decoder_layer, num_layers, norm=None, return_intermediate=False, d_model=256):
        super().__init__()
        self.layers = _get_clones(decoder_layer, num_layers)
        self.num_layers = num_layers
        self.norm = norm
        self.return_intermediate = return_intermediate
        self.d_model = d_model
        self.query_scale = MLP(d_model, d_model, d_model, 2)
        self.ref_point_head = MLP(d_model, d_model, 2, 2)
        for layer_id in range(num_layers - 1):
            self.layers[layer_id + 1].ca_qpos_proj = None

    def _memory_side_all(self, memory, pos, mem_cache):
        mem_w = [m for layer in self.layers for m in (layer.ca_kcontent_proj, layer.ca_v_proj)]
        pos_w = [layer.ca_kpos_proj for layer in self.layers]
        Wm, bm = [m.weight for m in mem_w], [m.bias for m in mem_w]
        Wp, bp = [m.weight for m in pos_w], [m.bias for m in pos_w]
        if not (memory.is_cuda and ops.multi_linear_ok(memory, Wm, bm) and ops.multi_linear_ok(pos, Wp, bp)):
            return
        B, S, d = memory.shape
        H, dh = self.layers[0].nhead, d // self.layers[0].nhead
        if ops.memory_side_kv_ok(memory, Wm, Wp, H):
            holder, toks = ops.memory_side_kv(memory, pos, H, Wm, Wp, bm, bp)
            for l in range(len(self.layers)):
                mem_cache[l] = (holder, toks[l], l)
            return
        ym = ops.multi_linear(memory, Wm, bm)
        yp = ops.multi_linear(pos, Wp, bp)
        for l in range(len(self.layers)):
            kc, v, kp = ym[2 * l], ym[2 * l + 1], yp[l]
            k = kc + kp if l == 0 else kc
            k = torch.cat([k.view(B, S, H, dh), kp.view(B, S, H, dh)], dim=3)
            mem_cache[l] = (k.view(B, S, 2 * d), v)

    def _query_pos_all(self, query_pos):
        mods = [m for layer in self.layers for m in (layer.sa_qpos_proj, layer.sa_kpos_proj)] + [self.layers[0].ca_qpos_proj]
        if not ops.group_linear_ok(query_pos, mods[:2]):
            return None
        outs = []
        for i in range(0, len(mods), 16):
            chunk = mods[i:i + 16]
            outs += list(ops.group_linear(query_pos, chunk)) if len(chunk) > 1 else [chunk[0](query_pos)]
        return [(outs[2 * l], outs[2 * l + 1], outs[-1] if l == 0 else None) for l in range(len(self.layers))]

    def forward(self, tgt, memory, memory_key_padding_mask, pos, query_pos, mem_cache=None, n_stages=1):
        mem_cache = {} if mem_cache is None else mem_cache
        output = tgt
        reference_points = self.ref_point_head(query_pos).sigmoid()
        intermediate = []
        sine0 = gen_sineembed_for_position(reference_points[..., :2], self.d_model)
        if not mem_cache:
            self._memory_side_all(memory, pos, mem_cache)
        qp_all = self._query_pos_all(query_pos)
        for layer_id, layer in enumerate(self.layers):
            if layer_id not in mem_cache:
                mem_cache[layer_id] = layer.memory_side(memory, pos, layer_id == 0)
            sine = sine0
            if layer_id > 0:
                sine = sine0 * self.query_scale(output)
            output = layer(output, mem_cache[layer_id], memory_key_padding_mask, query_pos, sine, layer_id == 0,
                           n_stages=n_stages, qp=None if qp_all is None else qp_all[layer_id])
            intermediate.append(self.norm(output))
        return torch.stack(intermediate), reference_points


class Transformer(nn.Module):
    def __init__(self, d_model=512, nhead=8, num_queries=300, num_encoder_layers=6, num_decoder_layers=6,
                 dim_feedforward=2048, dropout=0.1, activation="relu", normalize_before=False,
                 return_intermediate_dec=False, args=None, num_refines=1, drloc=False):
        super().__init__()
        enc_layer = TransformerEncoderLayer(d_model, nhead, dim_feedforward, dropout, activation, normalize_before)
        self.encoder = TransformerEncoder(enc_layer, num_encoder_layers, None)
        dec_layer = TransformerDecoderLayer(d_model, nhead, dim_feedforward, dropout, activation, normalize_before)
        self.decoder = TransformerDecoder(dec_layer, num_decoder_layers, LayerNorm(d_model),
                                          return_intermediate=return_intermediate_dec, d_model=d_model)
        self.H = self.W = None
        self._reset_parameters()
        self.d_model, self.nhead = d_model, nhead
        self.dec_layers, self.num_queries, self.num_refines = num_decoder_layers, num_queries, num_refines

    def _reset_parameters(self):
        for p in self.parameters():
            if p.dim() > 1:
                nn.init.xavier_uniform_(p)

    def forward(self, src, mask, query_embed, pos_embed, queries_embed_refine=None):
        B = src.shape[0]
        memory = src.flatten(2).transpose(1, 2).contiguous()
        pos = pos_embed.flatten(2).transpose(1, 2).contiguous()
        mask = mask.flatten(1)
        memory = self.encoder(memory, src_key_padding_mask=mask, pos=pos)
        queries = [query_embed] + [qe.weight for qe in (queries_embed_refine or [])]
        R, Q = len(queries), query_embed.shape[0]
        query_pos = torch.stack(queries).reshape(1, R * Q, -1).expand(B, -1, -1).contiguous()
        h, r = self.decoder(torch.zeros_like(query_pos), memory, mask, pos, query_pos, n_stages=R)
        hs = [h[:, :, i * Q:(i + 1) * Q] for i in range(R)]
        refs = [r[:, i * Q:(i + 1) * Q] for i in range(R)]
        return hs, refs


def _get_clones(module, n):
    return nn.ModuleList([copy.deepcopy(module) for _ in range(n)])


def build_transformer(args):
    return Transformer(d_model=args.hidden_dim, dropout=args.dropout, nhead=args.nheads, num_queries=args.num_queries,
                       dim_feedforward=args.dim_feedforward, num_encoder_layers=args.enc_layers,
                       num_decoder_layers=args.dec_layers, normalize_before=args.pre_norm, return_intermediate_dec=True)
```

### spe_amd/ops.py

```python
import os

import torch
from torch.autograd import Function

from . import kernels as K

ACT_NONE, ACT_RELU, ACT_GELU = 0, 1, 2


class _Linear(Function):

    @staticmethod
    @K.forward_scope
    def forward(ctx, x, W, b, act):
        shp = x.shape
        x2 = x.reshape(-1, shp[-1])
        if not x2.is_contiguous():
            x2 = x2.contiguous()
        Wc = W if W.is_contiguous() else W.contiguous()
        y, pre, xsave = K.linear_fwd(x2, Wc, b, act, want_pre=(act == ACT_GELU), save_for_dw=ctx.needs_input_grad[1], src=x)
        aux = pre if act == ACT_GELU else (y if act == ACT_RELU else None)
        ctx.act = act
        ctx.has_bias = b is not None
        ctx.params = (W, b)
        ctx.save_for_backward(xsave, Wc, aux)
        return y.view(*shp[:-1], W.shape[0])

    @staticmethod
    @K.backward_scope
    def backward(ctx, dy):
        x2, W, aux = ctx.saved_tensors
        dy2 = dy.reshape(-1, W.shape[0])
        if not dy2.is_contiguous():
            dy2 = dy2.contiguous()
        Wp, bp = ctx.params
        need_dw, need_db = ctx.needs_input_grad[1], ctx.has_bias and ctx.needs_input_grad[2]
        dx, dW, db = K.linear_bwd(dy2, x2, W, ctx.needs_input_grad[0], need_dw, need_db,
                                  dW_out=K.grad_buffer(Wp) if need_dw and Wp.is_contiguous() else None,
                                  db_out=K.grad_buffer(bp) if need_db else None, act=ctx.act, act_aux=aux)
        if dx is not None:
            dx = dx.view(*dy.shape[:-1], W.shape[1])
        return dx, dW, db, None


def linear(x, W, b=None, act=ACT_NONE):
    return _Linear.apply(x, W, b, act)


class _MultiLinear(Function):

    @staticmethod
    @K.forward_scope
    def forward(ctx, x, *wb):
        n = len(wb) // 2
        Ws, bs = wb[:n], wb[n:]
        shp = x.shape
        x2 = x.reshape(-1, shp[-1])
        if not x2.is_contiguous():
            x2 = x2.contiguous()
        R, Kd = x2.shape
        N = Ws[0].shape[0]
        sp = K.split_fwd()
        cat = K.weightcat16(Ws, bs, lo=sp)
        Wc, WcT, bc = cat[:3]
        x16, x16lo = K.act16(x2, x, want_lo=sp)
        y = torch.empty((R, n * N), device=x.device, dtype=torch.float32)
        K.gemm16(x16, Wc, y, R, n * N, Kd, Kd, Kd, n * N, bias=bc, Alo=x16lo, Blo=cat[3] if sp else None)
        ctx.params = (Ws, bs)
        ctx.save_for_backward(x16, WcT)
        ctx.dims = (n, N, Kd, R)
        y = y.view(*shp[:-1], n * N)
        return tuple(y[..., i * N:(i + 1) * N] for i in range(n))

    @staticmethod
    @K.backward_scope
    def backward(ctx, *dys):
        x16, WcT = ctx.saved_tensors
        n, N, Kd, R = ctx.dims
        Ws, bs = ctx.params
        dev = x16.device
        dy16 = torch.empty((R, n * N), device=dev, dtype=torch.bfloat16)
        dWs, dbs = [], []
        for i in range(n):
            blk = dy16[:, i * N:(i + 1) * N]
            if dys[i] is None:
                blk.zero_()
                dWs.append(None); dbs.append(None)
                continue
            d2 = dys[i].reshape(R, N)
            if not d2.is_contiguous():
                d2 = d2.contiguous()
            db = K._zeros_or(K.grad_buffer(bs[i]), N, dev)
            K.cvt_bf16(d2, True, False, colsum_out=db, out=blk, ldo=n * N)
            dbs.append(db)
            dWs.append(K._dw16_tn(blk, x16, N, Kd, R, K.grad_buffer(Ws[i]), lda=n * N))
        dx = None
        if ctx.needs_input_grad[0]:
            dx = torch.empty((R, Kd), device=dev, dtype=torch.float32)
            K.gemm16(dy16, WcT, dx, R, Kd, n * N, n * N, n * N, Kd)
            dx = dx.view(*dys[0].shape[:-1], Kd) if dys[0] is not None else dx
        return (dx, *dWs, *dbs)


def multi_linear_ok(x, Ws, bs):
    R = x.numel() // x.shape[-1]
    N, Kd = Ws[0].shape
    return (K._lin16_ok(R, len(Ws) * N, Kd) and all(W.shape == Ws[0].shape and W.is_contiguous() for W in Ws)
            and all(b is not None for b in bs) and N % 8 == 0)


def multi_linear(x, Ws, bs):
    return _MultiLinear.apply(x, *Ws, *bs)


class _GroupLinear(Function):

    @staticmethod
    @K.forward_scope
    def forward(ctx, x, n_add, *rest):
        adds, wb = rest[:n_add], rest[n_add:]
        n = len(wb) // 2
        Ws, bs = wb[:n], wb[n:]
        shp = x.shape
        x2 = x.reshape(-1, shp[-1])
        if not x2.is_contiguous():
            x2 = x2.contiguous()
        N = Ws[0].shape[0]
        a2 = None
        if n_add:
            a2 = [None if a is None else (lambda u: u if u.is_contiguous() else u.contiguous())(a.reshape(-1, N)) for a in adds]
        ys, x16 = K.linear_group_fwd(x2, Ws, bs, src=x, adds=a2)
        ctx.set_materialize_grads(False)
        ctx.params = (Ws, bs)
        ctx.add_shapes = tuple(None if a is None else a.shape for a in adds)
        ctx.save_for_backward(x16)
        return tuple(y.view(*shp[:-1], N) for y in ys)

    @staticmethod
    @K.backward_scope
    def backward(ctx, *dys):
        (x16,) = ctx.saved_tensors
        Ws, bs = ctx.params
        n, N = len(Ws), Ws[0].shape[0]
        d2 = []
        for d in dys:
            if d is None:
                d2.append(None)
                continue
            d = d.reshape(-1, N)
            d2.append(d if d.is_contiguous() else d.contiguous())
        dx, dWs, dbs = K.linear_group_bwd(d2, x16, Ws, ctx.needs_input_grad[0],
                                          [K.grad_buffer(W) if d is not None else None for W, d in zip(Ws, d2)],
                                          [K.grad_buffer(b) if d is not None else None for b, d in zip(bs, d2)])
        if dx is not None:
            ref = next(d for d in dys if d is not None)
            dx = dx.view(*ref.shape[:-1], Ws[0].shape[1])
        dadds = tuple(None if (shp is None or d is None) else d.reshape(shp) for shp, d in zip(ctx.add_shapes, dys))
        return (dx, None, *dadds, *dWs, *[None if b is None else b.view_as(p) for b, p in zip(dbs, bs)])


def group_linear_ok(x, mods):
    if not x.is_cuda or len(mods) < 2:
        return False
    R = x.numel() // x.shape[-1]
    return K.linear_group_ok(R, [m.weight for m in mods], [m.bias for m in mods])


def group_linear(x, mods, adds=None):
    adds = tuple(adds) if adds is not None else ()
    assert len(adds) in (0, len(mods))
    return _GroupLinear.apply(x, len(adds), *adds, *[m.weight for m in mods], *[m.bias for m in mods])


class _LayerNorm(Function):
    @staticmethod
    @K.forward_scope
    def forward(ctx, x, g, b, eps):
        x2 = x.reshape(-1, x.shape[-1])
        if not x2.is_contiguous():
            x2 = x2.contiguous()
        y, mean, rstd = K.layernorm_fwd(x2, g, b, eps)
        ctx.params = (g, b)
        ctx.save_for_backward(x2, g, mean, rstd)
        return y.view(x.shape)

    @staticmethod
    @K.backward_scope
    def backward(ctx, dy):
        x2, g, mean, rstd = ctx.saved_tensors
        dy2 = dy.reshape(-1, dy.shape[-1])
        if not dy2.is_contiguous():
            dy2 = dy2.contiguous()
        gp, bp = ctx.params
        dx, dg, db = K.layernorm_bwd(dy2, x2, g, mean, rstd, dg_out=K.grad_buffer(gp), db_out=K.grad_buffer(bp))
        return dx.view(dy.shape), dg.view_as(gp), db.view_as(bp), None


def layer_norm(x, g, b, eps):
    return _LayerNorm.apply(x, g, b, eps)


class _ResDropLayerNorm(Function):

    @staticmethod
    @K.forward_scope
    def forward(ctx, x, z, g, b, eps, p):
        x2 = x.reshape(-1, x.shape[-1])
        z2 = z.reshape(-1, z.shape[-1])
        x2 = x2 if x2.is_contiguous() else x2.contiguous()
        z2 = z2 if z2.is_contiguous() else z2.contiguous()
        seed, off = K.next_rng() if p > 0 else (0, 0)
        y, sm, mean, rstd = K.layernorm_res_fwd(x2, z2, g, b, eps, p, seed, off)
        ctx.params = (g, b)
        ctx.drop = (p, seed, off)
        ctx.save_for_backward(sm, g, mean, rstd)
        return y.view(x.shape)

    @staticmethod
    @K.backward_scope
    def backward(ctx, dy):
        sm, g, mean, rstd = ctx.saved_tensors
        dy2 = dy.reshape(-1, dy.shape[-1])
        dy2 = dy2 if dy2.is_contiguous() else dy2.contiguous()
        gp, bp = ctx.params
        p, seed, off = ctx.drop
        ds, dz, dg, db = K.layernorm_res_bwd(dy2, sm, g, mean, rstd, p, seed, off, dg_out=K.grad_buffer(gp), db_out=K.grad_buffer(bp))
        return ds.view(dy.shape), dz.view(dy.shape), dg.view_as(gp), db.view_as(bp), None, None


def res_drop_layer_norm(x, z, g, b, eps, p, training):
    return _ResDropLayerNorm.apply(x, z, g, b, eps, p if training else 0.0)


class _ResDropLayerNorm2(Function):

    @staticmethod
    @K.forward_scope
    def forward(ctx, x, z, g, b, eps, p):
        x2 = x.reshape(-1, x.shape[-1])
        z2 = z.reshape(-1, z.shape[-1])
        x2 = x2 if x2.is_contiguous() else x2.contiguous()
        z2 = z2 if z2.is_contiguous() else z2.contiguous()
        seed, off = K.next_rng() if p > 0 else (0, 0)
        y, sm, mean, rstd = K.layernorm_res_fwd(x2, z2, g, b, eps, p, seed, off)
        ctx.params = (g, b)
        ctx.drop = (p, seed, off)
        ctx.save_for_backward(sm, g, mean, rstd)
        yv = y.view(x.shape)
        return yv, yv.view_as(yv)

    @staticmethod
    @K.backward_scope
    def backward(ctx, dy, dy_b):
        sm, g, mean, rstd = ctx.saved_tensors
        if dy is None:
            dy, dy_b = dy_b, None
        if dy is None:
            return None, None, None, None, None, None
        c2 = lambda t: None if t is None else (lambda u: u if u.is_contiguous() else u.contiguous())(t.reshape(-1, t.shape[-1]))
        gp, bp = ctx.params
        p, seed, off = ctx.drop
        ds, dz, dg, db = K.layernorm_res_bwd(c2(dy), sm, g, mean, rstd, p, seed, off, dg_out=K.grad_buffer(gp), db_out=K.grad_buffer(bp), dy_b=c2(dy_b))
        return ds.view(dy.shape), dz.view(dy.shape), dg.view_as(gp), db.view_as(bp), None, None


def res_drop_layer_norm2(x, z, g, b, eps, p, training):
    return _ResDropLayerNorm2.apply(x, z, g, b, eps, p if training else 0.0)


class _LayerNormSkip(Function):

    @staticmethod
    @K.forward_scope
    def forward(ctx, x, g, b, eps, f16=False):
        x2 = x.reshape(-1, x.shape[-1])
        if not x2.is_contiguous():
            x2 = x2.contiguous()
        if K.produces16(*x2.shape):
            y, mean, rstd, y16, y16lo = K.layernorm_fwd(x2, g, b, eps, want16=True, f16=f16)
            yv = y.view(x.shape)
            K.attach16(yv, y16, y16lo)
        else:
            y, mean, rstd = K.layernorm_fwd(x2, g, b, eps)
            yv = y.view(x.shape)
        ctx.params = (g, b)
        prod = x.grad_fn if (K.LN_LS_FUSE and x.requires_grad) else None
        ctx.prod = prod if (prod is not None and getattr(prod, "ls_single", False) and x2.shape[1] <= 512) else None
        ctx.save_for_backward(x2, g, mean, rstd)
        return yv, x.view_as(x)

    @staticmethod
    @K.backward_scope
    def backward(ctx, dy, dskip):
        x2, g, mean, rstd = ctx.saved_tensors
        gp, bp = ctx.params
        if dy is None:
            return dskip, None, None, None, None
        dy2 = dy.reshape(-1, dy.shape[-1])
        if not dy2.is_contiguous():
            dy2 = dy2.contiguous()
        add = None
        if dskip is not None:
            add = dskip.reshape(-1, dskip.shape[-1])
            if not add.is_contiguous():
                add = add.contiguous()
        prod = ctx.prod
        if prod is not None:
            yls, gls, bpar, gpar = _ls_args(prod)
            dx, dg, db, done = K.layernorm_bwd(dy2, x2, g, mean, rstd, dg_out=K.grad_buffer(gp), db_out=K.grad_buffer(bp), add=add,
                                               ls=(yls, gls, K.grad_buffer(bpar), K.grad_buffer(gpar)))
            dxv = dx.view(dy.shape)
            prod.ls_done = (done, dx.data_ptr(), dxv._version)
            return dxv, dg.view_as(gp), db.view_as(bp), None, None
        dx, dg, db = K.layernorm_bwd(dy2, x2, g, mean, rstd, dg_out=K.grad_buffer(gp), db_out=K.grad_buffer(bp), add=add)
        return dx.view(dy.shape), dg.view_as(gp), db.view_as(bp), None, None


def layer_norm_skip(x, g, b, eps, f16=False):
    return _LayerNormSkip.apply(x, g, b, eps, f16)


class _LayerScaleResidual(Function):

    @staticmethod
    @K.forward_scope
    def forward(ctx, x, y, gamma, sample_scale):
        B = x.shape[0]
        x2 = x.reshape(-1, x.shape[-1]).contiguous()
        y2 = y.reshape(-1, y.shape[-1]).contiguous()
        rps = x2.shape[0] // B
        out = K.layerscale_residual_fwd(x2, y2, gamma, sample_scale, rps)
        ctx.rps = rps
        ctx.gamma = gamma
        ctx.save_for_backward(y2, gamma, sample_scale)
        return out.view(x.shape)

    @staticmethod
    @K.backward_scope
    def backward(ctx, dout):
        y2, gamma, ss = ctx.saved_tensors
        d2 = dout.reshape(-1, dout.shape[-1]).contiguous()
        dy, dg = K.layerscale_residual_bwd(d2, y2, gamma, ss, ctx.rps, dg_out=K.grad_buffer(ctx.gamma))
        return dout, dy.view(dout.shape), dg.view_as(ctx.gamma), None


def layerscale_residual(x, y, gamma, sample_scale=None):
    return _LayerScaleResidual.apply(x, y, gamma, sample_scale)


def drop_path_scale(B, p, training, device):
    if p <= 0.0 or not training:
        return None
    keep = 1.0 - p
    return (torch.rand(B, device=device) < keep).to(torch.float32) / keep


class _Dropout(Function):
    @staticmethod
    @K.forward_scope
    def forward(ctx, x, p):
        seed, off = K.next_rng()
        ctx.p, ctx.seed, ctx.off = p, seed, off
        return K.dropout(x.contiguous(), p, seed, off)

    @staticmethod
    @K.backward_scope
    def backward(ctx, dy):
        return K.dropout(dy.contiguous(), ctx.p, ctx.seed, ctx.off), None


def dropout(x, p, training):
    if p <= 0.0 or not training:
        return x
    return _Dropout.apply(x, p)


class _TalkingHeadsAttention(Function):

    @staticmethod
    @K.forward_scope
    def forward(ctx, qkv, Wl, bl, Ww, bw, H, scale, p_drop, acc=None):
        B, N, C3 = qkv.shape
        C = C3 // 3
        dh = C // H
        qkv = qkv.contiguous()
        v5 = qkv.view(B, N, 3, H, dh)
        q, k, v = v5[:, :, 0], v5[:, :, 1], v5[:, :, 2]
        ld = K.pad4(N)
        S = torch.empty((B, H, N, ld), device=qkv.device, dtype=torch.float32)
        sq = (N * C3, dh)
        sS = (H * N * ld, N * ld)
        K.gemm(q, k, S, N, N, dh, C3, C3, ld, False, True, batch0=B, batch1=H, sA=sq, sB=sq, sC=sS, alpha=scale)
        seed, off = K.next_rng() if p_drop > 0 else (0, 0)
        P, Pd = K.talking_fwd(S, Wl, bl, Ww, bw, B, H, N, N, ld, p_drop, seed, off)
        if acc is not None:
            K.attn_pmean_dense(P, acc[0], acc[1], B, H, N, ld)
        O = torch.empty((B, N, C), device=qkv.device, dtype=torch.float32)
        K.gemm(Pd, v, O, N, dh, N, ld, C3, C, False, False, batch0=B, batch1=H, sA=sS, sB=sq, sC=(N * C, dh))
        ctx.meta = (B, N, C, H, dh, ld, scale, p_drop, seed, off)
        ctx.save_for_backward(qkv, P, Pd, Wl, Ww)
        return O

    @staticmethod
    @K.backward_scope
    def backward(ctx, dO):
        qkv, P, Pd, Wl, Ww = ctx.saved_tensors
        B, N, C, H, dh, ld, scale, p_drop, seed, off = ctx.meta
        C3 = 3 * C
        dO = dO.contiguous()
        v5 = qkv.view(B, N, 3, H, dh)
        q, k, v = v5[:, :, 0], v5[:, :, 1], v5[:, :, 2]
        dqkv = torch.empty_like(qkv)
        d5 = dqkv.view(B, N, 3, H, dh)
        dq, dk, dv = d5[:, :, 0], d5[:, :, 1], d5[:, :, 2]
        sq, sS, sO = (N * C3, dh), (H * N * ld, N * ld), (N * C, dh)
        dPd = torch.empty((B, H, N, ld), device=qkv.device, dtype=torch.float32)
        K.gemm(dO, v, dPd, N, N, dh, C, C3, ld, False, True, batch0=B, batch1=H, sA=sO, sB=sq, sC=sS)
        K.gemm(Pd, dO, dv, N, dh, N, ld, C, C3, True, False, batch0=B, batch1=H, sA=sS, sB=sO, sC=sq)
        S = torch.empty((B, H, N, ld), device=qkv.device, dtype=torch.float32)
        K.gemm(q, k, S, N, N, dh, C3, C3, ld, False, True, batch0=B, batch1=H, sA=sq, sB=sq, sC=sS, alpha=scale)
        dS, dWl, dbl, dWw, dbw = K.talking_bwd(dPd, P, S, Wl, Ww, B, H, N, N, ld, p_drop, seed, off)
        del S
        K.gemm(dS, k, dq, N, dh, N, ld, C3, C3, False, False, batch0=B, batch1=H, sA=sS, sB=sq, sC=sq, alpha=scale)
        K.gemm(dS, q, dk, N, dh, N, ld, C3, C3, True, False, batch0=B, batch1=H, sA=sS, sB=sq, sC=sq, alpha=scale)
        return dqkv, dWl, dbl, dWw, dbw, None, None, None, None


class _TalkingHeadsAttentionFused(Function):

    @staticmethod
    @K.forward_scope
    def forward(ctx, qkv, Wl, bl, Ww, bw, H, scale, p_drop, acc=None):
        train = any(ctx.needs_input_grad)
        O, saved = _TalkingHeadsAttentionFused._fwd(ctx, qkv, Wl, bl, Ww, bw, H, scale, p_drop, train, acc)
        if train:
            ctx.save_for_backward(*saved)
        return O

    @staticmethod
    def _fwd(ctx, qkv, Wl, bl, Ww, bw, H, scale, p_drop, train, acc=None):
        B, N, C3 = qkv.shape
        C = C3 // 3
        dh = C // H
        qkv = qkv.contiguous()
        v5 = qkv.view(B, N, 3, H, dh)
        q, k, v = v5[:, :, 0], v5[:, :, 1], v5[:, :, 2]
        nt = (N + 15) // 16
        jobs = [(q, scale * K.LOG2E, 32 + K.F16), (k, 1.0, 32 + K.F16), (v, 1.0, 16 + K.F16)]
        if train:
            jobs += [(v, 1.0, 32), (k, 1.0, 16), (q, 1.0, 16)]
        packed = K.attn_pack_multi(jobs)
        Qf, Kf, V16 = packed[:3]
        Wl, bl, Ww, bw = Wl.contiguous(), bl.contiguous(), Ww.contiguous(), bw.contiguous()
        seed, off = K.next_rng() if p_drop > 0 else (0, 0)
        _, _, c0 = K.talking_row_constants(Qf, Kf, Wl, bl, B, H, N, dh)
        want16 = K.produces16(B * N, C)
        if acc is not None:
            K.attn_pmean(Qf, Kf, Wl, c0, acc[0], acc[1], B, H, N, dh)
        O, O16, O16lo, bits = K.talking_flash_fwd(Qf, Kf, V16, Wl, Ww, bw, c0, B, H, N, dh, p_drop, seed, off, want16, K.split_fwd(),
                                                  want_bits=True)
        if O16 is not None:
            K.attach16(O, O16, O16lo)
        ctx.meta = (B, N, C, H, dh, nt, scale, p_drop)
        ctx.wparams = (Wl, bl, Ww, bw)
        ctx.has_bits = train and bits is not None
        saved = (packed[3], packed[4], packed[5], Qf, Kf, c0, Wl, Ww, bw) + ((bits,) if ctx.has_bits else ()) if train else ()
        return O, saved

    @staticmethod
    @K.backward_scope
    def backward(ctx, dO):
        return (*_TalkingHeadsAttentionFused._bwd(ctx, ctx.saved_tensors, dO, False), None, None, None, None)

    @staticmethod
    def _bwd(ctx, saved, dO, out16):
        Vf, K16, Q16, Qf, Kf, c0, Wl, Ww, bw = saved[:9]
        kbits = saved[9] if ctx.has_bits else None
        B, N, C, H, dh, nt, scale, p_drop = ctx.meta
        dO = dO.contiguous()
        dqkv = torch.empty((B, N, 3 * C), device=dO.device, dtype=torch.bfloat16 if out16 else torch.float32)
        d5 = dqkv.view(B, N, 3, H, dh)
        dq, dk, dv = d5[:, :, 0], d5[:, :, 1], d5[:, :, 2]
        f32 = (lambda t: None) if out16 else (lambda t: t)
        b16 = (lambda t: t) if out16 else (lambda t: None)
        dO4 = dO.view(B, N, H, dh)
        dOf, dO16 = K.attn_pack_multi([(dO4, 1.0, 32), (dO4, 1.0, 16)])
        dS = K.score_blocks(B, H, N, dO.device)
        Drows, ws_w = K.talking_bwdk_pass1(Qf, dOf, dO16, Kf, Vf, Wl, Ww, bw, c0, kbits, f32(dv), b16(dv), B, H, N, dh, p_drop)
        K.talking_bwdq_pass2(Qf, dOf, Kf, Vf, K16, Wl, Ww, c0, Drows, ws_w, dS, f32(dq), b16(dq), scale, kbits, B, H, N, dh, p_drop)
        dWl, dbl, dWw, dbw = K.talking_wgrad_reduce(ws_w, H, ctx.wparams)
        K.attn_contract(dS, Q16, f32(dk), True, alpha=scale, out16=b16(dk))
        return dqkv, dWl, dbl, dWw, dbw


class _QkvTalkingAttention(Function):

    @staticmethod
    @K.forward_scope
    def forward(ctx, x, Wq, bq, Wl, bl, Ww, bw, H, scale, p_drop, acc=None):
        shp = x.shape
        x2 = x.reshape(-1, shp[-1])
        if not x2.is_contiguous():
            x2 = x2.contiguous()
        y, _, xsave = K.linear_fwd(x2, Wq, bq, 0, want_pre=False, save_for_dw=True, src=x)
        O, saved = _TalkingHeadsAttentionFused._fwd(ctx, y.view(*shp[:-1], Wq.shape[0]), Wl, bl, Ww, bw, H, scale, p_drop, True, acc)
        ctx.qparams = (Wq, bq)
        ctx.save_for_backward(xsave, *saved)
        return O

    @staticmethod
    @K.backward_scope
    def backward(ctx, dO):
        xsave, *saved = ctx.saved_tensors
        Wq, bq = ctx.qparams
        d16, dWl, dbl, dWw, dbw = _TalkingHeadsAttentionFused._bwd(ctx, saved, dO, True)
        N3, Kd = Wq.shape
        R = d16.numel() // N3
        d16 = d16.view(R, N3)
        dev = d16.device
        gb = K.grad_buffer(bq)
        db = gb.view(-1) if gb is not None else torch.empty((N3,), device=dev, dtype=torch.float32)
        K.colsum_bf16_blocks(d16, N3, [db])
        dW = K._dw16_tn(d16, xsave, N3, Kd, R, K.grad_buffer(Wq)) if ctx.needs_input_grad[1] else None
        dx = None
        if ctx.needs_input_grad[0]:
            dx = torch.empty((R, Kd), device=dev, dtype=torch.float32)
            K.gemm16(d16, K.weight16(Wq)[1], dx, R, Kd, N3, N3, N3, Kd)
            dx = dx.view(*dO.shape[:-1], Kd)
        return dx, dW, db.view_as(bq), dWl, dbl, dWw, dbw, None, None, None, None


def qkv_talking_attention_ok(x, Wq, bq, num_heads):
    C = x.shape[-1]
    R = x.numel() // C
    return (x.is_cuda and bq is not None and Wq.is_contiguous() and torch.is_grad_enabled()
            and (x.requires_grad or Wq.requires_grad) and Wq.requires_grad and bq.requires_grad
            and K.get_precision() != "bf16x3" and K._lin16_ok(R, Wq.shape[0], C) and not K._lin_small_ok(R, Wq.shape[0], C)
            and K.fused_supported(num_heads, C // num_heads))


def qkv_talking_attention(x, Wq, bq, Wl, bl, Ww, bw, num_heads, scale, p_drop=0.0, acc=None):
    return _QkvTalkingAttention.apply(x, Wq, bq, Wl, bl, Ww, bw, num_heads, scale, p_drop, acc)


class _MlpGelu(Function):

    @staticmethod
    @K.forward_scope
    def forward(ctx, x, W1, b1, W2, b2):
        shp = x.shape
        x2 = x.reshape(-1, shp[-1])
        if not x2.is_contiguous():
            x2 = x2.contiguous()
        train = any(ctx.needs_input_grad)
        y, saved = K.mlp_gelu_fwd(x2, W1, b1, W2, b2, save=train, src=x)
        ctx.params = (W1, b1, W2, b2)
        if train:
            ctx.save_for_backward(*saved, W1, W2)
        return y.view(*shp[:-1], W2.shape[0])

    @staticmethod
    @K.backward_scope
    def backward(ctx, dy):
        x16, pre, h16, W1, W2 = ctx.saved_tensors
        dy2 = dy.reshape(-1, W2.shape[0])
        if not dy2.is_contiguous():
            dy2 = dy2.contiguous()
        bufs = tuple(K.grad_buffer(p) for p in ctx.params)
        dx, dW1, db1, dW2, db2 = K.mlp_gelu_bwd(dy2, (x16, pre, h16), W1, W2, ctx.needs_input_grad[0], bufs)
        return (dx.view(*dy.shape[:-1], W1.shape[1]) if dx is not None else None), dW1, db1, dW2, db2


class _LinearRes(Function):

    @staticmethod
    @K.forward_scope
    def forward(ctx, x, W, b, xres, gamma, sscale=None, p_drop=0.0, single=False):
        shp = x.shape
        x2 = x.reshape(-1, shp[-1])
        if not x2.is_contiguous():
            x2 = x2.contiguous()
        r2 = xres.reshape(-1, xres.shape[-1])
        if not r2.is_contiguous():
            r2 = r2.contiguous()
        train = any(ctx.needs_input_grad)
        ctx.drop = (float(p_drop), *K.next_rng()) if p_drop > 0 else None
        ctx.ls_single = bool(single and train and p_drop <= 0 and sscale is None and not K.MLP_PRE_F16 and W.requires_grad
                             and b.requires_grad and gamma.requires_grad)
        ctx.ls_done = None
        ctx.rps = r2.shape[0] // xres.shape[0]
        out, saved = K.linear_res_fwd(x2, W, b, r2, gamma, save=train, src=x, drop=ctx.drop, sscale=sscale, rps=ctx.rps)
        ctx.params = (W, b, gamma)
        ctx.has_ss = sscale is not None
        if train:
            ctx.save_for_backward(*saved, W, gamma, *((sscale,) if sscale is not None else ()))
        return out.view(xres.shape)

    @staticmethod
    @K.backward_scope
    def backward(ctx, dout):
        x16, y, W, gamma = ctx.saved_tensors[:4]
        ss = ctx.saved_tensors[4] if ctx.has_ss else None
        d2 = dout.reshape(-1, W.shape[0])
        if not d2.is_contiguous():
            d2 = d2.contiguous()
        pre = _ls_taken(ctx, dout if dout.is_contiguous() else d2)
        bufs = tuple(K.grad_buffer(p) for p in ctx.params)
        dx, dW, db, dg = K.linear_res_bwd(d2, (x16, y), W, gamma, ctx.needs_input_grad[0], bufs, drop=ctx.drop, sscale=ss, rps=ctx.rps, pre=pre)
        return (dx.view(*dout.shape[:-1], W.shape[1]) if dx is not None else None), dW, db, dout, dg.view_as(gamma), None, None, None

def _ls_args(prod):
    sv = prod.saved_tensors
    if prod._forward_cls is _LinearRes:
        return sv[1], sv[3], prod.params[1], prod.params[2]
    return sv[3], sv[6], prod.params[3], prod.params[4]


def _ls_taken(ctx, d2):
    done = getattr(ctx, "ls_done", None)
    if done is None:
        return None
    ctx.ls_done = None
    pre, ptr, ver = done
    if d2.data_ptr() != ptr or d2._version != ver:
        raise RuntimeError("spe_amd.ops: a node was marked single=True but its output had more than one consumer (the LayerNorm backward already "
                           "accumulated its bias / LayerScale gradients from a partial gradient)")
    return pre


FUSE_DROP = True


def linear_residual(x, W, b, xres, gamma, sample_scale=None, p_drop=0.0, single=False):
    R = x.numel() // x.shape[-1]
    N, Kd = W.shape
    if ((FUSE_DROP or (sample_scale is None and p_drop <= 0)) and b is not None and W.is_contiguous()
            and gamma.is_contiguous() and N % 4 == 0 and N <= 1024 and K._lin16_ok(R, N, Kd)
            and (sample_scale is None or (sample_scale.is_contiguous() and R % xres.shape[0] == 0))):
        return _LinearRes.apply(x, W, b, xres, gamma, sample_scale, p_drop, single)
    return layerscale_residual(xres, dropout(linear(x, W, b), p_drop, p_drop > 0), gamma, sample_scale)


class _MlpGeluRes(Function):

    @staticmethod
    @K.forward_scope
    def forward(ctx, x, W1, b1, W2, b2, xres, gamma, sscale=None, p_drop=0.0, single=False):
        shp = x.shape
        x2 = x.reshape(-1, shp[-1])
        if not x2.is_contiguous():
            x2 = x2.contiguous()
        r2 = xres.reshape(-1, xres.shape[-1])
        if not r2.is_contiguous():
            r2 = r2.contiguous()
        train = any(ctx.needs_input_grad)
        ctx.drop1 = (float(p_drop), *K.next_rng()) if p_drop > 0 else None
        ctx.drop2 = (float(p_drop), *K.next_rng()) if p_drop > 0 else None
        ctx.ls_single = bool(single and train and p_drop <= 0 and sscale is None and not K.MLP_PRE_F16 and W2.requires_grad
                             and b2.requires_grad and gamma.requires_grad)
        ctx.ls_done = None
        ctx.rps = r2.shape[0] // xres.shape[0]
        out, saved = K.mlp_gelu_fwd(x2, W1, b1, W2, b2, res=r2, gamma=gamma, save=train, src=x, drop1=ctx.drop1, drop2=ctx.drop2,
                                    sscale=sscale, rps=ctx.rps)
        ctx.params = (W1, b1, W2, b2, gamma)
        ctx.has_ss = sscale is not None
        if train:
            ctx.save_for_backward(*saved, W1, W2, gamma, *((sscale,) if sscale is not None else ()))
        return out.view(xres.shape)

    @staticmethod
    @K.backward_scope
    def backward(ctx, dout):
        x16, pre, h16, y, W1, W2, gamma = ctx.saved_tensors[:7]
        ss = ctx.saved_tensors[7] if ctx.has_ss else None
        d2 = dout.reshape(-1, W2.shape[0])
        if not d2.is_contiguous():
            d2 = d2.contiguous()
# ... 465 lines not shown
```

Before: 42.50 images/sec.

## Fuse decoder query projection, FFN relu-dropout, and sine embedding into custom kernels

Adds three fused paths in the conditional-DETR decoder. The first projects content and scaled sine queries into their interleaved per-head halves in one kernel, with the query_scale multiply folded in. The second is a linear+ReLU+dropout kernel that applies the dropout mask in the GEMM epilogue, and its backward folds in the ReLU/dropout scaling. The third is a dedicated sine positional embedding kernel. Together they remove separate elementwise kernels, torch.cat copies and intermediate tensors on these small decoder tensors, at the cost of more complex kernels and a different dropout RNG stream.

```diff
diff --git a/include/spe_hip.h b/include/spe_hip.h
--- a/include/spe_hip.h
+++ b/include/spe_hip.h
@@ -48,9 +48,19 @@
                          void* x16_out, int R, int N, int K, long ldc, int act, spe_stream_t stream);
 int spe_linear_small_bwd(const float* dy, const float* aux, int act, const void* x16, const void* WT16, float* dx, float* dW,
                          float* db, int R, int N, int K, spe_stream_t stream);
+int spe_linear_small_drop_fwd(const float* x, long ldx, const void* W16, const void* W16lo, const float* bias, float* y, void* x16_out,
+                              int R, int N, int K, int act, float p, uint64_t seed, uint64_t offset, spe_stream_t stream);
+int spe_linear_small_drop_bwd(const float* dy, const float* yd, float p, const void* x16, const void* WT16, float* dx, float* dW,
+                              float* db, int R, int N, int K, spe_stream_t stream);
 int spe_linear_small_group_fwd(const float* x, long ldx, const void* const* W16, const void* const* W16lo, const float* const* bias,
                                const float* const* add, float* const* y, void* x16_out, int R, int nblk, int N, int K, spe_stream_t stream);
 int spe_linear_small_group_bwd(const float* const* dy, const void* x16, const void* const* WT16, float* dx, float* const* dW,
+                               float* const* db, int R, int nblk, int N, int K, spe_stream_t stream);
+int spe_linear_small_place_fwd(const float* const* x, const float* const* mul, const void* const* W16, const void* const* W16lo,
+                               const float* const* bias, const float* const* add, const long* add_place, float* y, const long* y_place,
+                               void* const* x16_out, int R, int nblk, int N, int K, spe_stream_t stream);
+int spe_linear_small_place_bwd(const float* const* dy, const long* dy_place, const void* const* x16, const void* const* WT16,
+                               const float* const* x, const float* const* mul, float* const* dx, float* const* dmul, float* const* dW,
                                float* const* db, int R, int nblk, int N, int K, spe_stream_t stream);
 int spe_gemm_bf16tn(const void* A16, const void* B16, float* C, int M, int N, int R, long lda, long ldb, long ldc,
                     float alpha, int splitk, spe_stream_t stream);
@@ -193,6 +203,9 @@
 int spe_pos_learned_fwd(const float* col, const float* row, float* out, int B, int h, int w, int npf, spe_stream_t stream);
 int spe_pos_learned_bwd(const float* g, float* d_col, float* d_row, int B, int h, int w, int npf, spe_stream_t stream);
 
+int spe_sine_embed_fwd(const float* pos, const float* dim_t, float* out, long R, int npf, float scale, spe_stream_t stream);
+int spe_sine_embed_bwd(const float* g, const float* pos, const float* dim_t, float* dpos, long R, int npf, float scale, spe_stream_t stream);
+
 int spe_nms_sorted(const float* boxes, const long* labels, const int* counts, unsigned char* keep, int nimg, int nmax,
                    float iou_threshold, spe_stream_t stream);
 
diff --git a/spe_amd/csrc/linear_small.hip b/spe_amd/csrc/linear_small.hip
--- a/spe_amd/csrc/linear_small.hip
+++ b/spe_amd/csrc/linear_small.hip
@@ -16,6 +16,7 @@
     const float* aux; int act;
     const unsigned short* xs16;
     float* dW; float* db;
+    float dscale;
     int R, N, K, tiles_dx;
     int nblk, Nblk;
     const unsigned short* Wb[LS_MAXBLK]; const unsigned short* Wlob[LS_MAXBLK]; const float* biasb[LS_MAXBLK]; float* yb[LS_MAXBLK];
@@ -23,8 +24,15 @@
     const float* dyb[LS_MAXBLK]; const unsigned short* WTb[LS_MAXBLK]; float* dWb[LS_MAXBLK]; float* dbb[LS_MAXBLK];
 };
 
-__device__ __forceinline__ float ls_dact(float v, float h, int act) {
+struct LsExt {
+    const float* mul;
+    int hw, hstride;
+};
+__device__ __forceinline__ long ls_place(int c, int hw, int hstride) { return hw > 0 ? (long)(c / hw) * hstride + c % hw : (long)c; }
+
+__device__ __forceinline__ float ls_dact(float v, float h, int act, float dscale = 1.f) {
     if (act == 1) return h > 0.f ? v : 0.f;
+    if (act == 3) return h > 0.f ? v * dscale : 0.f;
     if (act == 2) {
         const float cdf = 0.5f * (1.f + spe_erff(h * 0.70710678118654752f));
         const float pdf = 0.3989422804014327f * __expf(-0.5f * h * h);
@@ -37,11 +45,12 @@
     return __builtin_bit_cast(uint2, v);
 }
 
-template <int LS_KC, bool SPLIT, bool DACT>
+template <int LS_KC, bool SPLIT, bool DACT, bool EXT = false>
 __device__ __forceinline__ void ls_nt_tile(const float* __restrict__ A, long lda, const float* __restrict__ aux, int act, int r0, int R,
                                            const unsigned short* __restrict__ B, const unsigned short* __restrict__ Blo, int n0, int N, int K,
                                            unsigned short* x16, bool write_x16, unsigned short* smem, f32x4_t& acc,
-                                           const float* const* Ab = nullptr, const unsigned short* const* Bb = nullptr, int Nblk = 0) {
+                                           const float* const* Ab = nullptr, const unsigned short* const* Bb = nullptr, int Nblk = 0, float dscale = 1.f,
+                                           const LsExt ext = LsExt{nullptr, 0, 0}) {
     constexpr int LS_LD = LS_KC + 8, LS_NA = LS_KC / 32, LS_NB = LS_KC / 64;
     unsigned short* sA = smem;
     unsigned short* sB = sA + LS_T * LS_LD;
@@ -49,7 +58,7 @@
     unsigned short* sBl = sAl + LS_T * LS_LD;
     const int t = threadIdx.x, lane = t & 63, w = t >> 6, wm = w >> 1, wn = w & 1, fr = lane & 15, fk = (lane >> 4) * 8;
     acc = (f32x4_t){0.f, 0.f, 0.f, 0.f};
-    float4 xa[LS_NA], ha[DACT ? LS_NA : 1];
+    float4 xa[LS_NA], ha[DACT ? LS_NA : 1], ma[EXT ? LS_NA : 1];
     u32x4g_t wb[LS_NB], wl[SPLIT ? LS_NB : 1];
     auto load = [&](int k0) {
         const int kw = min(LS_KC, K - k0), n4 = kw >> 2, n8 = kw >> 3;
@@ -59,7 +68,11 @@
         for (int i = 0; i < LS_NA; ++i) {
             const int rl = (t >> 5) + 8 * (i & 3), c4 = (t & 31) + 32 * (i >> 2);
             if (c4 >= n4) continue;
-            const long off = (long)min(r0 + rl, R - 1) * lda_ + kk + c4 * 4;
+            long off = (long)min(r0 + rl, R - 1) * lda_ + kk + c4 * 4;
+            if constexpr (EXT) {
+                if (ext.mul) ma[i] = *reinterpret_cast<const float4*>(ext.mul + off);
+                off = (long)min(r0 + rl, R - 1) * lda_ + ls_place(kk + c4 * 4, ext.hw, ext.hstride);
+            }
             xa[i] = Ak ? *reinterpret_cast<const float4*>(Ak + off) : make_float4(0.f, 0.f, 0.f, 0.f);
             if constexpr (DACT) { if (aux) ha[i] = *reinterpret_cast<const float4*>(aux + off); }
         }
@@ -82,8 +95,11 @@
             if (c4 >= n4) continue;
             float4 v = xa[i];
             if (r0 + rl >= R) v = make_float4(0.f, 0.f, 0.f, 0.f);
+            if constexpr (EXT) {
+                if (ext.mul) { v.x *= ma[i].x; v.y *= ma[i].y; v.z *= ma[i].z; v.w *= ma[i].w; }
+            }
             if constexpr (DACT) {
-                if (aux) { v.x = ls_dact(v.x, ha[i].x, act); v.y = ls_dact(v.y, ha[i].y, act); v.z = ls_dact(v.z, ha[i].z, act); v.w = ls_dact(v.w, ha[i].w, act); }
+                if (aux) { v.x = ls_dact(v.x, ha[i].x, act, dscale); v.y = ls_dact(v.y, ha[i].y, act, dscale); v.z = ls_dact(v.z, ha[i].z, act, dscale); v.w = ls_dact(v.w, ha[i].w, act, dscale); }
             }
             bf16x4l_t h; h[0] = (__bf16)v.x; h[1] = (__bf16)v.y; h[2] = (__bf16)v.z; h[3] = (__bf16)v.w;
             const uint2 uh = __builtin_bit_cast(uint2, h);
@@ -121,6 +137,21 @@
         }
         if (k0 + LS_KC < K) __syncthreads();
     }
+}
+
+__device__ __forceinline__ void ls_epilogue_drop(const Gemm16Args& p, const f32x4_t& acc, const int m0, const int n0) {
+    const int lane = threadIdx.x & 63, w = threadIdx.x >> 6;
+    const int m = m0 + (w >> 1) * 16 + (lane & 15), n = n0 + (w & 1) * 16 + (lane >> 4) * 4;
+    if (m >= p.M || n >= p.N) return;
+    float v[4], ks[4];
+#pragma unroll
+    for (int r = 0; r < 4; ++r) {
+        v[r] = acc[r] * p.alpha + (p.bias ? p.bias[n + r] : 0.f);
+        if (p.act == 1) v[r] = fmaxf(v[r], 0.f);
+        else if (p.act == 2) v[r] = gelu_erf16(v[r]);
+    }
+    spe_drop_scale4(p.drop_seed, p.drop_off, (uint64_t)m * (uint64_t)p.N + (uint64_t)n, p.drop_p, ks);
+    spe_store4_stream(p.C + (long)m * p.ldc + n, v[0] * ks[0], v[1] * ks[1], v[2] * ks[2], v[3] * ks[3]);
 }
 
 template <int KC, bool SPLIT>
@@ -149,6 +180,7 @@
     }
     ls_nt_tile<KC, SPLIT, false>(p.x, p.ldx, nullptr, 0, tr * LS_T, p.g.M, p.g.B, p.g.Blo, tn * LS_T, p.g.N, p.g.K, p.x16, p.x16 != nullptr && tn == 0,
                              ls_smem, acc1);
+    if (p.g.drop_p > 0.f) { ls_epilogue_drop(p.g, acc1, tr * LS_T, tn * LS_T); return; }
     f32x4_t acc[1][1] = {{acc1}};
     gemm16_epilogue_plain<LS_T, LS_T>(p.g, acc, p.g.C, tr * LS_T, tn * LS_T);
 }
@@ -162,9 +194,92 @@
     return __builtin_bit_cast(bf16x8_t, v);
 }
 
+template <int LS_RC, bool EXT>
+__device__ __forceinline__ void ls_tn_tile(const float* __restrict__ dyp, long ldy, int Nld, const float* __restrict__ aux, int act, float dscale,
+                                           const unsigned short* __restrict__ xs16, int n0, int k0, int R, int K, float* dWp, float* dbp,
+                                           unsigned short* ls_smem, const LsExt ext = LsExt{nullptr, 0, 0}) {
+    constexpr int LS_ND = LS_RC / 32, LS_NX = LS_RC / 64;
+    const int t = threadIdx.x, lane = t & 63, w = t >> 6, wm = w >> 1, wn = w & 1, fr = lane & 15;
+    unsigned short* sD = ls_smem;
+    unsigned short* sX = sD + LS_RC * LS_LDT;
+    float* sred = reinterpret_cast<float*>(sX + LS_RC * LS_LDT);
+    const bool want_dw = dWp != nullptr, want_db = dbp != nullptr;
+    f32x4_t acc = {0.f, 0.f, 0.f, 0.f};
+    float4 bsum = make_float4(0.f, 0.f, 0.f, 0.f);
+    float4 dv[LS_ND], hv[LS_ND]; u32x4g_t xv[LS_NX];
+    auto load = [&](int rc0) {
+        const int cn = n0 + (t & 7) * 4, ck = k0 + (t & 3) * 8;
+        long coff = min(cn, Nld - 4);
+        if constexpr (EXT) coff = ls_place(min(cn, Nld - 4), ext.hw, ext.hstride);
+#pragma unroll
+        for (int i = 0; i < LS_ND; ++i) {
+            const int r = rc0 + (t >> 3) + 32 * i;
+            if (r >= R) continue;
+            const long off = (long)min(r, R - 1) * ldy + coff;
+            dv[i] = *reinterpret_cast<const float4*>(dyp + off);
+            if (aux) hv[i] = *reinterpret_cast<const float4*>(aux + off);
+        }
+        if (want_dw) {
+#pragma unroll
+            for (int i = 0; i < LS_NX; ++i) {
+                const int r = rc0 + (t >> 2) + 64 * i;
+                if (r >= R) continue;
+                xv[i] = *reinterpret_cast<const u32x4g_t*>(xs16 + (long)min(r, R - 1) * K + min(ck, K - 8));
+            }
+        }
+    };
+    load(0);
+    for (int rc0 = 0; rc0 < R; rc0 += LS_RC) {
+        const int rows = min(LS_RC, R - rc0), rpad = (rows + 31) & ~31;
+        const bool cnv = n0 + (t & 7) * 4 < Nld, ckv = k0 + (t & 3) * 8 < K;
+#pragma unroll
+        for (int i = 0; i < LS_ND; ++i) {
+            const int rl = (t >> 3) + 32 * i;
+            if (rl >= rpad) continue;
+            float4 v = dv[i];
+            if (aux) { v.x = ls_dact(v.x, hv[i].x, act, dscale); v.y = ls_dact(v.y, hv[i].y, act, dscale); v.z = ls_dact(v.z, hv[i].z, act, dscale); v.w = ls_dact(v.w, hv[i].w, act, dscale); }
+            if (rl >= rows || !cnv) v = make_float4(0.f, 0.f, 0.f, 0.f);
+            bsum.x += v.x; bsum.y += v.y; bsum.z += v.z; bsum.w += v.w;
+            *reinterpret_cast<uint2*>(sD + rl * LS_LDT + (t & 7) * 4) = ls_pack4(v.x, v.y, v.z, v.w);
+        }
+        if (want_dw) {
+#pragma unroll
+            for (int i = 0; i < LS_NX; ++i) {
+                const int rl = (t >> 2) + 64 * i;
+                if (rl >= rpad) continue;
+                *reinterpret_cast<u32x4g_t*>(sX + rl * LS_LDT + (t & 3) * 8) = (rl < rows && ckv) ? xv[i] : (u32x4g_t){0u, 0u, 0u, 0u};
+            }
+        }
+        if (rc0 + LS_RC < R) load(rc0 + LS_RC);
+        __syncthreads();
+        if (want_dw) {
+            for (int ks = 0; ks < rpad / 32; ++ks) {
+                const bf16x8_t a = ls_operand_t(sD, ks, wm * 16, lane);
+                const bf16x8_t b = ls_operand_t(sX, ks, wn * 16, lane);
+                acc = __builtin_amdgcn_mfma_f32_16x16x32_bf16(b, a, acc, 0, 0, 0);
+            }
+        }
+        if (rc0 + LS_RC < R) __syncthreads();
+    }
+    if (want_dw) {
+        const int n = n0 + wm * 16 + fr, k = k0 + wn * 16 + (lane >> 4) * 4;
+        if (n < Nld && k < K) *reinterpret_cast<float4*>(dWp + (long)n * K + k) = make_float4(acc[0], acc[1], acc[2], acc[3]);
+    }
+    if (want_db) {
+        __syncthreads();
+        *reinterpret_cast<float4*>(sred + (t >> 3) * 32 + (t & 7) * 4) = bsum;
+        __syncthreads();
+        if (t < LS_T && n0 + t < Nld) {
+            float s = 0.f;
+#pragma unroll
+            for (int i = 0; i < 32; ++i) s += sred[i * 32 + t];
+            dbp[n0 + t] = s;
+        }
+    }
+}
+
 template <int KC, int LS_RC>
 __global__ __launch_bounds__(256) void linear_small_bwd_kernel(LinSmallArgs p) {
-    constexpr int LS_ND = LS_RC / 32, LS_NX = LS_RC / 64;
     extern __shared__ __attribute__((aligned(16))) unsigned short ls_smem[];
     const int R = p.R, N = p.N, K = p.K;
     const int t = threadIdx.x, lane = t & 63, w = t >> 6, wm = w >> 1, wn = w & 1, fr = lane & 15;
@@ -174,14 +289,12 @@
         f32x4_t acc1;
         if (p.nblk > 0) ls_nt_tile<KC, false, true>(nullptr, 0, nullptr, 0, tr * LS_T, R, nullptr, nullptr, tk * LS_T, K, N, nullptr, false, ls_smem, acc1,
                                                     p.dyb, p.WTb, p.Nblk);
-        else ls_nt_tile<KC, false, true>(p.x, N, p.aux, p.act, tr * LS_T, R, p.g.B, nullptr, tk * LS_T, K, N, nullptr, false, ls_smem, acc1);
+        else ls_nt_tile<KC, false, true>(p.x, N, p.aux, p.act, tr * LS_T, R, p.g.B, nullptr, tk * LS_T, K, N, nullptr, false, ls_smem, acc1,
+                                         nullptr, nullptr, 0, p.dscale);
         const int r = tr * LS_T + wm * 16 + fr, k = tk * LS_T + wn * 16 + (lane >> 4) * 4;
         if (r < R && k < K) *reinterpret_cast<float4*>(p.g.C + (long)r * K + k) = make_float4(acc1[0], acc1[1], acc1[2], acc1[3]);
         return;
     }
-    unsigned short* sD = ls_smem;
-    unsigned short* sX = sD + LS_RC * LS_LDT;
-    float* sred = reinterpret_cast<float*>(sX + LS_RC * LS_LDT);
     const int b2 = blockIdx.x - p.tiles_dx;
     const int tiles_n = (N + LS_T - 1) / LS_T;
     const int tn = b2 % tiles_n, tk = b2 / tiles_n;
@@ -193,77 +306,7 @@
         dyp = p.dyb[blk]; dWp = p.dWb[blk]; dbp = p.dbb[blk];
         if (!dyp) return;
     }
-    const bool want_dw = dWp != nullptr, want_db = dbp != nullptr && tk == 0;
-    f32x4_t acc = {0.f, 0.f, 0.f, 0.f};
-    float4 bsum = make_float4(0.f, 0.f, 0.f, 0.f);
-    float4 dv[LS_ND], hv[LS_ND]; u32x4g_t xv[LS_NX];
-    auto load = [&](int rc0) {
-        const int cn = n0 + (t & 7) * 4, ck = k0 + (t & 3) * 8;
-#pragma unroll
-        for (int i = 0; i < LS_ND; ++i) {
-            const int r = rc0 + (t >> 3) + 32 * i;
-            if (r >= R) continue;
-            const long off = (long)min(r, R - 1) * Nld + min(cn, Nld - 4);
-            dv[i] = *reinterpret_cast<const float4*>(dyp + off);
-            if (p.aux) hv[i] = *reinterpret_cast<const float4*>(p.aux + off);
-        }
-        if (want_dw) {
-#pragma unroll
-            for (int i = 0; i < LS_NX; ++i) {
-                const int r = rc0 + (t >> 2) + 64 * i;
-                if (r >= R) continue;
-                xv[i] = *reinterpret_cast<const u32x4g_t*>(p.xs16 + (long)min(r, R - 1) * K + min(ck, K - 8));
-            }
-        }
-    };
-    load(0);
-    for (int rc0 = 0; rc0 < R; rc0 += LS_RC) {
-        const int rows = min(LS_RC, R - rc0), rpad = (rows + 31) & ~31;
-        const bool cnv = n0 + (t & 7) * 4 < Nld, ckv = k0 + (t & 3) * 8 < K;
-#pragma unroll
-        for (int i = 0; i < LS_ND; ++i) {
-            const int rl = (t >> 3) + 32 * i;
-            if (rl >= rpad) continue;
-            float4 v = dv[i];
-            if (p.aux) { v.x = ls_dact(v.x, hv[i].x, p.act); v.y = ls_dact(v.y, hv[i].y, p.act); v.z = ls_dact(v.z, hv[i].z, p.act); v.w = ls_dact(v.w, hv[i].w, p.act); }
-            if (rl >= rows || !cnv) v = make_float4(0.f, 0.f, 0.f, 0.f);
-            bsum.x += v.x; bsum.y += v.y; bsum.z += v.z; bsum.w += v.w;
-            *reinterpret_cast<uint2*>(sD + rl * LS_LDT + (t & 7) * 4) = ls_pack4(v.x, v.y, v.z, v.w);
-        }
-        if (want_dw) {
-#pragma unroll
-            for (int i = 0; i < LS_NX; ++i) {
-                const int rl = (t >> 2) + 64 * i;
-                if (rl >= rpad) continue;
-                *reinterpret_cast<u32x4g_t*>(sX + rl * LS_LDT + (t & 3) * 8) = (rl < rows && ckv) ? xv[i] : (u32x4g_t){0u, 0u, 0u, 0u};
-            }
-        }
-        if (rc0 + LS_RC < R) load(rc0 + LS_RC);
-        __syncthreads();
-        if (want_dw) {
-            for (int ks = 0; ks < rpad / 32; ++ks) {
-                const bf16x8_t a = ls_operand_t(sD, ks, wm * 16, lane);
-                const bf16x8_t b = ls_operand_t(sX, ks, wn * 16, lane);
-                acc = __builtin_amdgcn_mfma_f32_16x16x32_bf16(b, a, acc, 0, 0, 0);
-            }
-        }
-        if (rc0 + LS_RC < R) __syncthreads();
-    }
-    if (want_dw) {
-        const int n = n0 + wm * 16 + fr, k = k0 + wn * 16 + (lane >> 4) * 4;
-        if (n < Nld && k < K) *reinterpret_cast<float4*>(dWp + (long)n * K + k) = make_float4(acc[0], acc[1], acc[2], acc[3]);
-    }
-    if (want_db) {
-        __syncthreads();
-        *reinterpret_cast<float4*>(sred + (t >> 3) * 32 + (t & 7) * 4) = bsum;
-        __syncthreads();
-        if (t < LS_T && n0 + t < Nld) {
-            float s = 0.f;
-#pragma unroll
-            for (int i = 0; i < 32; ++i) s += sred[i * 32 + t];
-            dbp[n0 + t] = s;
-        }
-    }
+    ls_tn_tile<LS_RC, false>(dyp, Nld, Nld, p.aux, p.act, p.dscale, p.xs16, n0, k0, R, K, dWp, tk == 0 ? dbp : nullptr, ls_smem);
 }
 
 static int ls_latency_tiles() {
@@ -272,14 +315,15 @@
     return v;
 }
 
-extern "C" int spe_linear_small_fwd(const float* x, long ldx, const void* W16, const void* W16lo, const float* bias, float* y, float* pre,
-                                    void* x16_out, int R, int N, int K, long ldc, int act, hipStream_t stream) {
+static int ls_fwd_launch(const float* x, long ldx, const void* W16, const void* W16lo, const float* bias, float* y, float* pre,
+                         void* x16_out, int R, int N, int K, long ldc, int act, float drop_p, uint64_t seed, uint64_t offset, hipStream_t stream) {
     if (R <= 0 || N <= 0) return 0;
     auto al16 = [](const void* q) { return (reinterpret_cast<uintptr_t>(q) & 15) == 0; };
     if (K <= 0 || (K & 7) || (ldx & 3) || !al16(x) || !al16(W16) || !al16(W16lo) || !al16(x16_out)) return -2;
     LinSmallArgs p = {};
     p.g.B = reinterpret_cast<const unsigned short*>(W16); p.g.Blo = reinterpret_cast<const unsigned short*>(W16lo);
     p.g.C = y; p.g.C2 = pre; p.g.bias = bias; p.g.M = R; p.g.N = N; p.g.K = K; p.g.ldc = ldc; p.g.alpha = 1.f; p.g.act = act; p.g.splitk = 1;
+    p.g.drop_p = drop_p; p.g.drop_seed = seed; p.g.drop_off = offset;
     p.x = x; p.ldx = ldx; p.x16 = reinterpret_cast<unsigned short*>(x16_out);
     const int tiles = ((R + LS_T - 1) / LS_T) * ((N + LS_T - 1) / LS_T);
     const bool split = W16lo != nullptr;
@@ -303,14 +347,25 @@
     return 0;
 }
 
-extern "C" int spe_linear_small_bwd(const float* dy, const float* aux, int act, const void* x16, const void* WT16, float* dx, float* dW,
-                                    float* db, int R, int N, int K, hipStream_t stream) {
+extern "C" int spe_linear_small_fwd(const float* x, long ldx, const void* W16, const void* W16lo, const float* bias, float* y, float* pre,
+                                    void* x16_out, int R, int N, int K, long ldc, int act, hipStream_t stream) {
+    return ls_fwd_launch(x, ldx, W16, W16lo, bias, y, pre, x16_out, R, N, K, ldc, act, 0.f, 0, 0, stream);
+}
+
+extern "C" int spe_linear_small_drop_fwd(const float* x, long ldx, const void* W16, const void* W16lo, const float* bias, float* y,
+                                         void* x16_out, int R, int N, int K, int act, float p, uint64_t seed, uint64_t offset, hipStream_t stream) {
+    if (!(p >= 0.f && p < 1.f) || (N & 3) || (reinterpret_cast<uintptr_t>(y) & 15)) return -2;
+    return ls_fwd_launch(x, ldx, W16, W16lo, bias, y, nullptr, x16_out, R, N, K, N, act, p, seed, offset, stream);
+}
+
+static int ls_bwd_launch(const float* dy, const float* aux, int act, float dscale, const void* x16, const void* WT16, float* dx, float* dW,
+                         float* db, int R, int N, int K, hipStream_t stream) {
     if (R <= 0 || N <= 0 || K <= 0) return 0;
     auto al16 = [](const void* q) { return (reinterpret_cast<uintptr_t>(q) & 15) == 0; };
     if ((K & 7) || (N & 7) || !al16(dy) || !al16(aux) || !al16(x16) || !al16(WT16) || !al16(dx) || !al16(dW)) return -2;
-    if ((dx && !WT16) || (dW && !x16) || (aux && act != 1 && act != 2)) return -2;
+    if ((dx && !WT16) || (dW && !x16) || (aux && act != 1 && act != 2 && act != 3)) return -2;
     LinSmallArgs p = {};
-    p.x = dy; p.aux = aux; p.act = act; p.xs16 = reinterpret_cast<const unsigned short*>(x16);
+    p.x = dy; p.aux = aux; p.act = act; p.dscale = dscale; p.xs16 = reinterpret_cast<const unsigned short*>(x16);
     p.g.B = reinterpret_cast<const unsigned short*>(WT16); p.g.C = dx;
     p.dW = dW; p.db = db; p.R = R; p.N = N; p.K = K;
     const int tr = (R + LS_T - 1) / LS_T, tk = (K + LS_T - 1) / LS_T, tn = (N + LS_T - 1) / LS_T;
@@ -330,6 +385,18 @@
     else hipLaunchKernelGGL((linear_small_bwd_kernel<128, 256>), dim3(p.tiles_dx + tiles_dw), dim3(256), smem_of(128, 256), stream, p);
     SPE_CHECK_LAUNCH();
     return 0;
+}
+
+extern "C" int spe_linear_small_bwd(const float* dy, const float* aux, int act, const void* x16, const void* WT16, float* dx, float* dW,
+                                    float* db, int R, int N, int K, hipStream_t stream) {
+    if (R > 0 && N > 0 && K > 0 && aux && act != 1 && act != 2) return -2;
+    return ls_bwd_launch(dy, aux, act, 1.f, x16, WT16, dx, dW, db, R, N, K, stream);
+}
+
+extern "C" int spe_linear_small_drop_bwd(const float* dy, const float* yd, float p, const void* x16, const void* WT16, float* dx, float* dW,
+                                         float* db, int R, int N, int K, hipStream_t stream) {
+    if (!yd || !(p >= 0.f && p < 1.f)) return -2;
+    return ls_bwd_launch(dy, yd, 3, 1.0f / (1.0f - p), x16, WT16, dx, dW, db, R, N, K, stream);
 }
 
 static bool ls_group_kc_wide(int N) { return N % 384 == 0; }
@@ -405,3 +472,155 @@
     SPE_CHECK_LAUNCH();
     return 0;
 }
+
+#define LS_PLACE_MAXBLK 4
+struct LsPlacement { const float* base; long pitch; int coloff, hw, hstride; };
+struct LinPlaceArgs {
+    int R, N, K, nblk, tiles_dx;
+    const float* xb[LS_PLACE_MAXBLK]; const float* mulb[LS_PLACE_MAXBLK];
+    const unsigned short* Wb[LS_PLACE_MAXBLK]; const unsigned short* Wlob[LS_PLACE_MAXBLK]; const float* biasb[LS_PLACE_MAXBLK];
+    unsigned short* x16b[LS_PLACE_MAXBLK];
+    LsPlacement addb[LS_PLACE_MAXBLK]; LsPlacement yb[LS_PLACE_MAXBLK];
+    LsPlacement dyb[LS_PLACE_MAXBLK]; const unsigned short* WTb[LS_PLACE_MAXBLK]; const unsigned short* xs16b[LS_PLACE_MAXBLK];
+    float* dxb[LS_PLACE_MAXBLK]; float* dmulb[LS_PLACE_MAXBLK]; float* dWb[LS_PLACE_MAXBLK]; float* dbb[LS_PLACE_MAXBLK];
+};
+__device__ __forceinline__ long ls_placed(const LsPlacement& q, int m, int n) { return (long)m * q.pitch + q.coloff + ls_place(n, q.hw, q.hstride); }
+
+template <int KC, bool SPLIT>
+__global__ __launch_bounds__(256) void linear_place_fwd_kernel(LinPlaceArgs p) {
+    extern __shared__ __attribute__((aligned(16))) unsigned short ls_smem[];
+    const int tiles_r = (p.R + LS_T - 1) / LS_T, tpb = p.N / LS_T;
+    const int tr = blockIdx.x % tiles_r, tn = blockIdx.x / tiles_r, blk = tn / tpb, tl = tn - blk * tpb;
+    f32x4_t acc;
+    ls_nt_tile<KC, SPLIT, false, true>(p.xb[blk], p.K, nullptr, 0, tr * LS_T, p.R, p.Wb[blk], p.Wlob[blk], tl * LS_T, p.N, p.K, p.x16b[blk],
+                                       p.x16b[blk] != nullptr && tl == 0, ls_smem, acc, nullptr, nullptr, 0, 1.f, LsExt{p.mulb[blk], 0, 0});
+    const int lane = threadIdx.x & 63, w = threadIdx.x >> 6;
+    const int m = tr * LS_T + (w >> 1) * 16 + (lane & 15), n = tl * LS_T + (w & 1) * 16 + (lane >> 4) * 4;
+    if (m >= p.R) return;
+    float4 v = make_float4(acc[0], acc[1], acc[2], acc[3]);
+    if (p.biasb[blk]) v = spe_add4(v, *reinterpret_cast<const float4*>(p.biasb[blk] + n));
+    if (p.addb[blk].base) v = spe_add4(v, *reinterpret_cast<const float4*>(p.addb[blk].base + ls_placed(p.addb[blk], m, n)));
+    *reinterpret_cast<float4*>(const_cast<float*>(p.yb[blk].base) + ls_placed(p.yb[blk], m, n)) = v;
+}
+
+template <int KC, int LS_RC>
+__global__ __launch_bounds__(256) void linear_place_bwd_kernel(LinPlaceArgs p) {
+    extern __shared__ __attribute__((aligned(16))) unsigned short ls_smem[];
+    const int R = p.R, N = p.N, K = p.K;
+    const int tiles_r = (R + LS_T - 1) / LS_T, tiles_k = (K + LS_T - 1) / LS_T, tiles_n = N / LS_T;
+    if ((int)blockIdx.x < p.tiles_dx) {
+        const int blk = blockIdx.x / (tiles_r * tiles_k), b1 = blockIdx.x - blk * tiles_r * tiles_k;
+        const int tr = b1 % tiles_r, tk = b1 / tiles_r;
+        const LsPlacement& d = p.dyb[blk];
+        if (!d.base || !p.dxb[blk]) return;
+        f32x4_t acc;
+        ls_nt_tile<KC, false, true, true>(d.base + d.coloff, d.pitch, nullptr, 0, tr * LS_T, R, p.WTb[blk], nullptr, tk * LS_T, K, N, nullptr, false,
+                                          ls_smem, acc, nullptr, nullptr, 0, 1.f, LsExt{nullptr, d.hw, d.hstride});
+        const int t = threadIdx.x, lane = t & 63, w = t >> 6;
+        const int r = tr * LS_T + (w >> 1) * 16 + (lane & 15), k = tk * LS_T + (w & 1) * 16 + (lane >> 4) * 4;
+        if (r >= R || k >= K) return;
+        const long off = (long)r * K + k;
+        float4 v = make_float4(acc[0], acc[1], acc[2], acc[3]);
+        if (p.mulb[blk]) {
+            if (p.dmulb[blk]) *reinterpret_cast<float4*>(p.dmulb[blk] + off) = spe_mul4(v, *reinterpret_cast<const float4*>(p.xb[blk] + off));
+            v = spe_mul4(v, *reinterpret_cast<const float4*>(p.mulb[blk] + off));
+        }
+        *reinterpret_cast<float4*>(p.dxb[blk] + off) = v;
+        return;
+    }
+    const int b2 = blockIdx.x - p.tiles_dx;
+    const int blk = b2 / (tiles_n * tiles_k), b3 = b2 - blk * tiles_n * tiles_k;
+    const int tn = b3 % tiles_n, tk = b3 / tiles_n;
+    const LsPlacement& d = p.dyb[blk];
+    if (!d.base) return;
+    ls_tn_tile<LS_RC, true>(d.base + d.coloff, d.pitch, N, nullptr, 0, 1.f, p.xs16b[blk], tn * LS_T, tk * LS_T, R, K, p.dWb[blk],
+                            tk == 0 ? p.dbb[blk] : nullptr, ls_smem, LsExt{nullptr, d.hw, d.hstride});
+}
+
+static bool ls_place_ok(const long* q, int N) {
+    const long co = q[0], hw = q[1], hs = q[2], pitch = q[3];
+    return co >= 0 && hw > 0 && ((co | hw | hs | pitch) & 3) == 0 && N % hw == 0 && co + hw <= hs && (N / hw) * hs <= pitch && hs < (1L << 30);
+}
+static LsPlacement ls_placement(const float* base, const long* q) { return LsPlacement{base, q[3], (int)q[0], (int)q[1], (int)q[2]}; }
+
+extern "C" int spe_linear_small_place_fwd(const float* const* x, const float* const* mul, const void* const* W16, const void* const* W16lo,
+                                          const float* const* bias, const float* const* add, const long* add_place, float* y, const long* y_place,
+                                          void* const* x16_out, int R, int nblk, int N, int K, hipStream_t stream) {
+    if (R <= 0 || N <= 0 || nblk <= 0) return 0;
+    auto al16 = [](const void* q) { return (reinterpret_cast<uintptr_t>(q) & 15) == 0; };
+    if (nblk > LS_PLACE_MAXBLK || K <= 0 || (K & 7) || (N % LS_T) || !x || !W16 || !y || !y_place || !al16(y) || (add && !add_place)) return -2;
+    LinPlaceArgs p = {};
+    const bool split = W16lo != nullptr;
+    for (int i = 0; i < nblk; ++i) {
+        if (!x[i] || !W16[i] || !al16(x[i]) || !al16(W16[i]) || (split && (!W16lo[i] || !al16(W16lo[i]))) || !ls_place_ok(y_place + 4 * i, N)) return -2;
+        p.xb[i] = x[i]; p.mulb[i] = mul ? mul[i] : nullptr;
+        p.Wb[i] = reinterpret_cast<const unsigned short*>(W16[i]); p.Wlob[i] = split ? reinterpret_cast<const unsigned short*>(W16lo[i]) : nullptr;
+        p.biasb[i] = bias ? bias[i] : nullptr;
+        p.x16b[i] = x16_out ? reinterpret_cast<unsigned short*>(x16_out[i]) : nullptr;
+        p.yb[i] = ls_placement(y, y_place + 4 * i);
+        if (add && add[i]) {
+            if (!al16(add[i]) || !ls_place_ok(add_place + 4 * i, N)) return -2;
+            p.addb[i] = ls_placement(add[i], add_place + 4 * i);
+        }
+        if (!al16(p.mulb[i]) || !al16(p.biasb[i]) || !al16(p.x16b[i])) return -2;
+    }
+    p.R = R; p.N = N; p.K = K; p.nblk = nblk;
+    const int tiles = ((R + LS_T - 1) / LS_T) * (nblk * N / LS_T);
+    const bool wide = tiles <= ls_latency_tiles();
+    const int smem = (split ? 4 : 2) * LS_T * ((wide ? 384 : 128) + 8) * (int)sizeof(unsigned short);
+    static bool attr_set = false;
+    if (!attr_set) {
+        hipError_t e = hipFuncSetAttribute(reinterpret_cast<const void*>(&linear_place_fwd_kernel<384, true>), hipFuncAttributeMaxDynamicSharedMemorySize,
+                                           4 * LS_T * 392 * (int)sizeof(unsigned short));
+        if (e != hipSuccess) return (int)e;
+        attr_set = true;
+    }
+    if (wide) {
+        if (split) hipLaunchKernelGGL((linear_place_fwd_kernel<384, true>), dim3(tiles), dim3(256), smem, stream, p);
+        else hipLaunchKernelGGL((linear_place_fwd_kernel<384, false>), dim3(tiles), dim3(256), smem, stream, p);
+    } else {
+        if (split) hipLaunchKernelGGL((linear_place_fwd_kernel<128, true>), dim3(tiles), dim3(256), smem, stream, p);
+        else hipLaunchKernelGGL((linear_place_fwd_kernel<128, false>), dim3(tiles), dim3(256), smem, stream, p);
+    }
+    SPE_CHECK_LAUNCH();
+    return 0;
+}
+
+extern "C" int spe_linear_small_place_bwd(const float* const* dy, const long* dy_place, const void* const* x16, const void* const* WT16,
+                                          const float* const* x, const float* const* mul, float* const* dx, float* const* dmul,
+                                          float* const* dW, float* const* db, int R, int nblk, int N, int K, hipStream_t stream) {
+    if (R <= 0 || N <= 0 || K <= 0 || nblk <= 0) return 0;
+    auto al16 = [](const void* q) { return (reinterpret_cast<uintptr_t>(q) & 15) == 0; };
+    if (nblk > LS_PLACE_MAXBLK || (K & 7) || (N % LS_T) || !dy || !dy_place) return -2;
+    LinPlaceArgs p = {};
+    bool any_dx = false, any_dw = false;
+    for (int i = 0; i < nblk; ++i) {
+        if (!dy[i]) continue;
+        if (!al16(dy[i]) || !ls_place_ok(dy_place + 4 * i, N)) return -2;
+        p.dyb[i] = ls_placement(dy[i], dy_place + 4 * i);
+        p.dxb[i] = dx ? dx[i] : nullptr; p.WTb[i] = WT16 ? reinterpret_cast<const unsigned short*>(WT16[i]) : nullptr;
+        p.mulb[i] = mul ? mul[i] : nullptr; p.xb[i] = x ? x[i] : nullptr; p.dmulb[i] = dmul ? dmul[i] : nullptr;
+        p.dWb[i] = dW ? dW[i] : nullptr; p.dbb[i] = db ? db[i] : nullptr; p.xs16b[i] = x16 ? reinterpret_cast<const unsigned short*>(x16[i]) : nullptr;
+        if ((p.dxb[i] && !p.WTb[i]) || (p.dWb[i] && !p.xs16b[i]) || (p.dmulb[i] && (!p.mulb[i] || !p.xb[i] || !p.dxb[i]))) return -2;
+        if (!al16(p.dxb[i]) || !al16(p.WTb[i]) || !al16(p.mulb[i]) || !al16(p.xb[i]) || !al16(p.dmulb[i]) || !al16(p.dWb[i]) || !al16(p.xs16b[i])) return -2;
+        any_dx = any_dx || p.dxb[i]; any_dw = any_dw || p.dWb[i] || p.dbb[i];
+    }
+    p.R = R; p.N = N; p.K = K; p.nblk = nblk;
+    const int tr = (R + LS_T - 1) / LS_T, tk = (K + LS_T - 1) / LS_T, tn = N / LS_T;
+    p.tiles_dx = any_dx ? nblk * tr * tk : 0;
+    const int tiles_dw = any_dw ? nblk * tn * tk : 0;
+    if (p.tiles_dx + tiles_dw == 0) return 0;
+    const bool wide = p.tiles_dx + tiles_dw <= ls_latency_tiles();
+    auto smem_of = [](int kc, int rc) { const int a = 2 * LS_T * (kc + 8) * 2, b = 2 * rc * LS_LDT * 2 + 32 * 32 * 4; return a > b ? a : b; };
+    static bool attr_set = false;
+    if (!attr_set) {
+        hipError_t e = hipFuncSetAttribute(reinterpret_cast<const void*>(&linear_place_bwd_kernel<384, 512>), hipFuncAttributeMaxDynamicSharedMemorySize,
+                                           smem_of(384, 512));
+        if (e != hipSuccess) return (int)e;
+        attr_set = true;
+    }
+    if (wide) hipLaunchKernelGGL((linear_place_bwd_kernel<384, 512>), dim3(p.tiles_dx + tiles_dw), dim3(256), smem_of(384, 512), stream, p);
+    else hipLaunchKernelGGL((linear_place_bwd_kernel<128, 256>), dim3(p.tiles_dx + tiles_dw), dim3(256), smem_of(128, 256), stream, p);
+    SPE_CHECK_LAUNCH();
+    return 0;
+}
diff --git a/spe_amd/csrc/sine_embed.hip b/spe_amd/csrc/sine_embed.hip
--- /dev/null
+++ b/spe_amd/csrc/sine_embed.hip
@@ -0,0 +1,52 @@
+#include "common.h"
+
+__global__ __launch_bounds__(256) void sine_embed_fwd_kernel(const float* __restrict__ pos, const float* __restrict__ dim_t,
+                                                             float* __restrict__ out, long R, int npf, float scale) {
+    const long total = R * 2 * npf;
+    for (long i = (long)blockIdx.x * 256 + threadIdx.x; i < total; i += (long)gridDim.x * 256) {
+        const int c2 = (int)(i % (2 * npf));
+        const long r = i / (2 * npf);
+        const int c = c2 < npf ? c2 : c2 - npf;
+        const float p = pos[2 * r + (c2 < npf ? 1 : 0)];
+        const float ps = p * scale;
+        const float a = ps / dim_t[c];
+        out[i] = (c & 1) ? cosf(a) : sinf(a);
+    }
+}
+
+__global__ __launch_bounds__(256) void sine_embed_bwd_kernel(const float* __restrict__ g, const float* __restrict__ pos,
+                                                             const float* __restrict__ dim_t, float* __restrict__ dpos, int npf, float scale) {
+    __shared__ float red[2][16];
+    const long r = blockIdx.x;
+    const float px = pos[2 * r] * scale, py = pos[2 * r + 1] * scale;
+    const float* gr = g + r * 2 * npf;
+    float sx = 0.f, sy = 0.f;
+    for (int c = threadIdx.x; c < npf; c += 256) {
+        const float dt = dim_t[c], w = scale / dt;
+        const float ay = py / dt, ax = px / dt;
+        const float dy = (c & 1) ? -sinf(ay) : cosf(ay), dx = (c & 1) ? -sinf(ax) : cosf(ax);
+        sy += gr[c] * (dy * w);
+        sx += gr[npf + c] * (dx * w);
+    }
+    sx = spe_block_sum(sx, red[0]);
+    sy = spe_block_sum(sy, red[1]);
+    if (threadIdx.x == 0) { dpos[2 * r] = sx; dpos[2 * r + 1] = sy; }
+}
+
+extern "C" int spe_sine_embed_fwd(const float* pos, const float* dim_t, float* out, long R, int npf, float scale, hipStream_t st) {
+    if (R < 0 || npf < 1 || !pos || !dim_t || !out) return -2;
+    if (R == 0) return 0;
+    long nb = (R * 2 * npf + 255) / 256; if (nb > 4096) nb = 4096;
+    hipLaunchKernelGGL(sine_embed_fwd_kernel, dim3((unsigned)nb), dim3(256), 0, st, pos, dim_t, out, R, npf, scale);
+    SPE_CHECK_LAUNCH();
+    return 0;
+}
+
+extern "C" int spe_sine_embed_bwd(const float* g, const float* pos, const float* dim_t, float* dpos, long R, int npf, float scale,
+                                  hipStream_t st) {
+    if (R < 0 || R > 0x7fffffffL || npf < 1 || !g || !pos || !dim_t || !dpos) return -2;
+    if (R == 0) return 0;
+    hipLaunchKernelGGL(sine_embed_bwd_kernel, dim3((unsigned)R), dim3(256), 0, st, g, pos, dim_t, dpos, npf, scale);
+    SPE_CHECK_LAUNCH();
+    return 0;
+}
diff --git a/spe_amd/kernels.py b/spe_amd/kernels.py
--- a/spe_amd/kernels.py
+++ b/spe_amd/kernels.py
@@ -745,6 +745,74 @@
           _ptr_array([0 if w is None else w.data_ptr() for w in dWs]), _ptr_array([0 if b is None else b.data_ptr() for b in dbs]),
           R, n, N, K, _st())
     return dx, dWs, dbs
+
+
+LINEAR_PLACE_MAX = 4
+
+
+def place_whole(N):
+    return (0, N, N, N)
+
+
+def place_half(N, H, second):
+    dh = N // H
+    return (dh if second else 0, dh, 2 * dh, 2 * N)
+
+
+def linear_place_ok(R, Ws, bs, hw):
+    N, K = Ws[0].shape
+    return (1 <= len(Ws) <= LINEAR_PLACE_MAX and _lin_small_ok(R, N, K) and N % 32 == 0 and hw % 4 == 0 and N % hw == 0
+            and all(W.shape == Ws[0].shape and W.is_contiguous() for W in Ws) and all(b is not None for b in bs))
+
+
+def _place_array(places):
+    flat = [int(v) for q in places for v in (q if q is not None else (0, 0, 0, 0))]
+    return (ctypes.c_long * len(flat))(*flat)
+
+
+def linear_place_fwd(xs, muls, Ws, bs, adds, add_places, y, y_places, srcs=None):
+    _chk(y, *xs, *Ws)
+    R, K = xs[0].shape
+    N = Ws[0].shape[0]
+    sp = split_fwd()
+    trip = [weight16(W, lo=sp) for W in Ws]
+    x16s, outs = [], []
+    for i, x in enumerate(xs):
+        src = srcs[i] if (srcs is not None and muls[i] is None) else None
+        ent = getattr(src, "_spe16", None) if src is not None else None
+        x16 = ent[1] if (ent is not None and ent[0] == src._version and ent[1].shape == x.shape) else None
+        if x16 is None:
+            x16 = torch.empty((R, K), device=x.device, dtype=torch.bfloat16)
+            outs.append(x16.data_ptr())
+            if src is not None:
+                attach16(src, x16)
+        else:
+            outs.append(0)
+        x16s.append(x16)
+    _call("spe_linear_small_place_fwd", _ptr_array([x.data_ptr() for x in xs]), _ptr_array([0 if m is None else m.data_ptr() for m in muls]),
+          _ptr_array([t_[0].data_ptr() for t_ in trip]), _ptr_array([t_[2].data_ptr() for t_ in trip]) if sp else None,
+          _ptr_array([b.data_ptr() for b in bs]), _ptr_array([0 if a is None else a.data_ptr() for a in adds]), _place_array(add_places),
+          _p(y), _place_array(y_places), _ptr_array(outs), R, len(xs), N, K, _st())
+    return x16s
+
+
+def linear_place_bwd(dys, dy_places, x16s, Ws, xs, muls, need_dx, need_dmul, dW_outs, db_outs):
+    n = len(Ws)
+    N, K = Ws[0].shape
+    R = x16s[0].shape[0]
+    dev = x16s[0].device
+    new = lambda *s: torch.empty(s, device=dev, dtype=torch.float32)
+    dxs, dmuls, dWs, dbs = [], [], [], []
+    for i in range(n):
+        live = dys[i] is not None
+        dxs.append(new(R, K) if live and need_dx[i] else None)
+        dmuls.append(new(R, K) if live and need_dmul[i] and muls[i] is not None else None)
+        dWs.append((dW_outs[i] if dW_outs[i] is not None else new(N, K)) if live else None)
+        dbs.append((db_outs[i].view(-1) if db_outs[i] is not None else new(N)) if live else None)
+    ptrs = lambda ts: _ptr_array([0 if t_ is None else t_.data_ptr() for t_ in ts])
+    _call("spe_linear_small_place_bwd", ptrs(dys), _place_array(dy_places), ptrs(x16s), _ptr_array([weight16(W)[1].data_ptr() for W in Ws]),
+          ptrs(xs), ptrs(muls), ptrs(dxs), ptrs(dmuls), ptrs(dWs), ptrs(dbs), R, n, N, K, _st())
+    return dxs, dmuls, dWs, dbs
 
 
 def linear_bwd(dy2, xsave, W, need_dx=True, need_dw=True, need_db=True, dW_out=None, db_out=None, act=0, act_aux=None):
@@ -792,6 +860,70 @@
     return dx, dW, db
 
 
+def linear_drop_ok(R, N, K):
+    return _lin_small_ok(R, N, K)
+
+
+def linear_drop_fwd(x2, W, b, act, p, seed, offset, save_for_dw=True, src=None):
+    _chk(x2, W, b)
+    R, K = x2.shape
+    N = W.shape[0]
+    yd = torch.empty((R, N), device=x2.device, dtype=torch.float32)
+    sp = split_fwd()
+    Wt = weight16(W, lo=sp)
+    ent = getattr(src, "_spe16", None) if src is not None else None
+    x16 = ent[1] if (ent is not None and ent[0] == src._version and ent[1].shape == x2.shape) else None
+    x16_out = None
+    if x16 is None and save_for_dw:
+        x16 = x16_out = torch.empty((R, K), device=x2.device, dtype=torch.bfloat16)
+        if src is not None:
+            attach16(src, x16)
+    _call("spe_linear_small_drop_fwd", _p(x2), x2.stride(0), _p(Wt[0]), _p(Wt[2] if sp else None), _p(b), _p(yd), _p(x16_out),
+          R, N, K, int(act), float(p), seed, offset, _st())
+    return yd, (x16 if save_for_dw else None)
+
+
+def linear_drop_bwd(dy2, yd, p, x16, W, need_dx=True, need_dw=True, need_db=True, dW_out=None, db_out=None):
+    _chk(dy2, yd, W)
+    R, N = dy2.shape
+    K = W.shape[1]
+    dev = dy2.device
+    dx = torch.empty((R, K), device=dev, dtype=torch.float32) if need_dx else None
+    dW = (dW_out if dW_out is not None else torch.empty((N, K), device=dev, dtype=torch.float32)) if need_dw else None
+    db = (db_out.view(-1) if db_out is not None else torch.empty((N,), device=dev, dtype=torch.float32)) if need_db else None
+    _call("spe_linear_small_drop_bwd", _p(dy2), _p(yd), float(p), _p(x16 if need_dw else None), _p(weight16(W)[1] if need_dx else None),
+          _p(dx), _p(dW), _p(db), R, N, K, _st())
+    return dx, dW, db
+
+
+_SINE_DIM_T = {}
+
+
+def sine_dim_t(npf, device):
+    key = (int(npf), str(device))
+    t = _SINE_DIM_T.get(key)
+    if t is None:
+        t = torch.arange(npf, dtype=torch.float32, device=device)
+        t = _SINE_DIM_T[key] = (10000 ** (2 * torch.div(t, 2, rounding_mode="floor") / 128)).contiguous()
+    return t
+
+
+def sine_embed_fwd(pos2, npf, scale):
+    _chk(pos2)
+    R = pos2.shape[0]
+    out = torch.empty((R, 2 * npf), device=pos2.device, dtype=torch.float32)
+    _call("spe_sine_embed_fwd", _p(pos2), _p(sine_dim_t(npf, pos2.device)), _p(out), R, npf, float(scale), _st())
+    return out
+
+
+def sine_embed_bwd(g2, pos2, npf, scale):
+    _chk(g2, pos2)
+    R = pos2.shape[0]
+    dpos = torch.empty((R, 2), device=pos2.device, dtype=torch.float32)
+    _call("spe_sine_embed_bwd", _p(g2), _p(pos2), _p(sine_dim_t(npf, pos2.device)), _p(dpos), R, npf, float(scale), _st())
+    return dpos
+
+
 def colsum(x2, out=None, accumulate=True):
     _chk(x2)
     R, C = x2.shape
diff --git a/spe_amd/models/transformer.py b/spe_amd/models/transformer.py
--- a/spe_amd/models/transformer.py
+++ b/spe_amd/models/transformer.py
@@ -116,7 +116,7 @@
         k = torch.cat([k.view(B, S, H, dh), k_pos.view(B, S, H, dh)], dim=3)
         return k.view(B, S, 2 * d), v
 
-    def forward(self, tgt, mem_kv, memory_key_padding_mask, query_pos, query_sine_embed, is_first, n_stages=1, qp=None):
+    def forward(self, tgt, mem_kv, memory_key_padding_mask, query_pos, query_sine_embed, is_first, n_stages=1, qp=None, sine_scale=None):
         B, RQ, d = tgt.shape
         H, dh = self.nhead, d // self.nhead
         Q = RQ // n_stages
@@ -131,25 +131,31 @@
         sa = lambda t: t.view(B * n_stages, Q, d)
         tgt2 = self.self_attn(sa(q), sa(k), sa(v))[0].view(B, RQ, d)
         tgt, tgt_skip = self.norm1.residual2(tgt, tgt2, self.dropout1)
-        q = self.ca_qcontent_proj(tgt)
-        if is_first:
-            q = q + (ca_pos if ca_pos is not None else self.ca_qpos_proj(query_pos))
-        qs = self.ca_qpos_sine_proj(query_sine_embed)
-        if isinstance(mem_kv[0], ops.MemoryKV):
-            holder, tok, layer_id = mem_kv
+        frag_kv = isinstance(mem_kv[0], ops.MemoryKV)
+        if is_first and ca_pos is None:
+            ca_pos = self.ca_qpos_proj(query_pos)
+        if frag_kv and ops.ca_query_ok(tgt, self.ca_qcontent_proj, self.ca_qpos_sine_proj, H):
+            q = ops.ca_query(tgt, query_sine_embed, sine_scale, ca_pos if is_first else None, is_first,
+                             self.ca_qcontent_proj, self.ca_qpos_sine_proj, H)
+        else:
+            q = self.ca_qcontent_proj(tgt)
             if is_first:
+                q = q + ca_pos
+            qs = self.ca_qpos_sine_proj(query_sine_embed if sine_scale is None else query_sine_embed * sine_scale)
+            if frag_kv and is_first:
                 qs = qs + q
             q = torch.cat([q.view(B, RQ, H, dh), qs.view(B, RQ, H, dh)], dim=3)
+        if frag_kv:
+            holder, tok, layer_id = mem_kv
             ca = self.cross_attn
             o = ops.cross_attention_kv(q, tok, holder, layer_id, memory_key_padding_mask, float(ca.head_dim) ** -0.5,
                                        ca.dropout if ca.training else 0.0)
             tgt2 = ca.out_proj(o)
         else:
-            q = torch.cat([q.view(B, RQ, H, dh), qs.view(B, RQ, H, dh)], dim=3).view(B, RQ, 2 * d)
             k, v = mem_kv
-            tgt2 = self.cross_attn(q, k, v, key_padding_mask=memory_key_padding_mask)[0]
+            tgt2 = self.cross_attn(q.view(B, RQ, 2 * d), k, v, key_padding_mask=memory_key_padding_mask)[0]
         tgt, tgt_skip = self.norm2.residual2(tgt_skip, tgt2, self.dropout2)
-        tgt2 = self.linear2(self.dropout(self.linear1(tgt, ops.ACT_RELU)))
+        tgt2 = self.linear2(ops.linear_relu_dropout(tgt, self.linear1.weight, self.linear1.bias, self.dropout.p, self.dropout.training))
         return self.norm3.residual(tgt_skip, tgt2, self.dropout3)
 
 
@@ -203,18 +209,18 @@
         output = tgt
         reference_points = self.ref_point_head(query_pos).sigmoid()
         intermediate = []
-        sine0 = gen_sineembed_for_position(reference_points[..., :2], self.d_model)
+        ref_xy = reference_points[..., :2]
+        sine0 = (ops.sine_embed(ref_xy, self.d_model) if ops.sine_embed_ok(ref_xy, self.d_model)
+                 else gen_sineembed_for_position(ref_xy, self.d_model))
         if not mem_cache:
             self._memory_side_all(memory, pos, mem_cache)
         qp_all = self._query_pos_all(query_pos)
         for layer_id, layer in enumerate(self.layers):
             if layer_id not in mem_cache:
                 mem_cache[layer_id] = layer.memory_side(memory, pos, layer_id == 0)
-            sine = sine0
-            if layer_id > 0:
-                sine = sine0 * self.query_scale(output)
-            output = layer(output, mem_cache[layer_id], memory_key_padding_mask, query_pos, sine, layer_id == 0,
-                           n_stages=n_stages, qp=None if qp_all is None else qp_all[layer_id])
+            scale = self.query_scale(output) if layer_id > 0 else None
+            output = layer(output, mem_cache[layer_id], memory_key_padding_mask, query_pos, sine0, layer_id == 0,
+                           n_stages=n_stages, qp=None if qp_all is None else qp_all[layer_id], sine_scale=scale)
             intermediate.append(self.norm(output))
         return torch.stack(intermediate), reference_points
 
diff --git a/spe_amd/ops.py b/spe_amd/ops.py
--- a/spe_amd/ops.py
+++ b/spe_amd/ops.py
@@ -1,3 +1,4 @@
+import math
 import os
 
 import torch
@@ -172,6 +173,65 @@
     return _GroupLinear.apply(x, len(adds), *adds, *[m.weight for m in mods], *[m.bias for m in mods])
 
 
+class _CaQuery(Function):
+
+    @staticmethod
+    @K.forward_scope
+    def forward(ctx, tgt, sine, scale, ca_pos, carry, Wc, bc, Ws, bs, H):
+        B, RQ, d = tgt.shape
+        N = Wc.shape[0]
+        two = lambda t: None if t is None else (lambda u: u if u.is_contiguous() else u.contiguous())(t.reshape(B * RQ, -1))
+        t2, s2, m2, a2 = two(tgt), two(sine), two(scale), two(ca_pos)
+        q = torch.empty((B, RQ, H, 2 * (N // H)), device=tgt.device, dtype=torch.float32)
+        first, second = K.place_half(N, H, False), K.place_half(N, H, True)
+        if carry:
+            xa = K.linear_place_fwd([t2], [None], [Wc], [bc], [a2], [K.place_whole(N)], q, [first], srcs=[tgt])
+            xb = K.linear_place_fwd([s2], [m2], [Ws], [bs], [q], [first], q, [second], srcs=[sine])
+            x16s = xa + xb
+        else:
+            x16s = K.linear_place_fwd([t2, s2], [None, m2], [Wc, Ws], [bc, bs], [a2, None], [K.place_whole(N), None], q, [first, second],
+                                      srcs=[tgt, sine])
+        ctx.set_materialize_grads(False)
+        ctx.dims = (B, RQ, d, N, H, bool(carry), ca_pos is not None)
+        ctx.params = (Wc, bc, Ws, bs)
+        ctx.save_for_backward(x16s[0], x16s[1], s2 if m2 is not None else None, m2)
+        return q
+
+    @staticmethod
+    @K.backward_scope
+    def backward(ctx, dq):
+        if dq is None:
+            return (None,) * 10
+        x16c, x16s, s2, m2 = ctx.saved_tensors
+        B, RQ, d, N, H, carry, has_pos = ctx.dims
+        Wc, bc, Ws, bs = ctx.params
+        dh = N // H
+        dq = dq if dq.is_contiguous() else dq.contiguous()
+        first, second = K.place_half(N, H, False), K.place_half(N, H, True)
+        dyc, pc = dq, first
+        if carry:
+            dyc, pc = (dq[..., :dh] + dq[..., dh:]).view(B * RQ, N), K.place_whole(N)
+        need = ctx.needs_input_grad
+        dxs, dmuls, dWs, dbs = K.linear_place_bwd([dyc, dq], [pc, second], [x16c, x16s], [Wc, Ws], [None, s2], [None, m2],
+                                                  [need[0], need[1]], [False, need[2]],
+                                                  [K.grad_buffer(Wc), K.grad_buffer(Ws)], [K.grad_buffer(bc), K.grad_buffer(bs)])
+        v = lambda t: None if t is None else t.view(B, RQ, d)
+        dpos = None
+        if has_pos and need[3]:
+            dpos = dyc.view(B, RQ, N) if carry else dq[..., :dh].reshape(B, RQ, N)
+        return (v(dxs[0]), v(dxs[1]), v(dmuls[1]), dpos, None, dWs[0], dbs[0].view_as(bc), dWs[1], dbs[1].view_as(bs), None)
+
+
+def ca_query_ok(tgt, mc, ms, H):
+    if not tgt.is_cuda or tgt.dim() != 3 or mc.weight.shape[0] % H:
+        return False
+    return K.linear_place_ok(tgt.shape[0] * tgt.shape[1], [mc.weight, ms.weight], [mc.bias, ms.bias], mc.weight.shape[0] // H)
+
+
+def ca_query(tgt, sine, scale, ca_pos, carry, mc, ms, H):
+    return _CaQuery.apply(tgt, sine, scale, ca_pos, carry, mc.weight, mc.bias, ms.weight, ms.bias, H)
+
+
 class _LayerNorm(Function):
     @staticmethod
     @K.forward_scope
@@ -373,6 +433,79 @@
     if p <= 0.0 or not training:
         return x
     return _Dropout.apply(x, p)
+
+
+class _LinearReluDropout(Function):
+
+    @staticmethod
+    @K.forward_scope
+    def forward(ctx, x, W, b, p):
+        shp = x.shape
+        x2 = x.reshape(-1, shp[-1])
+        if not x2.is_contiguous():
+            x2 = x2.contiguous()
+        seed, off = K.next_rng()
+        yd, x16 = K.linear_drop_fwd(x2, W, b, ACT_RELU, p, seed, off, save_for_dw=ctx.needs_input_grad[1], src=x)
+        ctx.p = p
+        ctx.has_bias = b is not None
+        ctx.params = (W, b)
+        ctx.save_for_backward(x16, W, yd)
+        return yd.view(*shp[:-1], W.shape[0])
+
+    @staticmethod
+    @K.backward_scope
+    def backward(ctx, dy):
+        x16, W, yd = ctx.saved_tensors
+        dy2 = dy.reshape(-1, W.shape[0])
+        if not dy2.is_contiguous():
+            dy2 = dy2.contiguous()
+        Wp, bp = ctx.params
+        need_dw, need_db = ctx.needs_input_grad[1], ctx.has_bias and ctx.needs_input_grad[2]
+        dx, dW, db = K.linear_drop_bwd(dy2, yd, ctx.p, x16, W, ctx.needs_input_grad[0], need_dw, need_db,
+                                       dW_out=K.grad_buffer(Wp) if need_dw else None, db_out=K.grad_buffer(bp) if need_db else None)
+        if dx is not None:
+            dx = dx.view(*dy.shape[:-1], W.shape[1])
+        return dx, dW, db, None
+
+
+def linear_relu_dropout(x, W, b, p, training):
+    if p <= 0.0 or not training:
+        return linear(x, W, b, ACT_RELU)
+    R = x.numel() // x.shape[-1]
+    if not (x.is_cuda and W.is_contiguous() and K.linear_drop_ok(R, W.shape[0], W.shape[1])):
+        return dropout(linear(x, W, b, ACT_RELU), p, training)
+    return _LinearReluDropout.apply(x, W, b, p)
+
+
+class _SineEmbed(Function):
+
+    @staticmethod
+    @K.forward_scope
+    def forward(ctx, pos, d_model):
+        npf = d_model // 2
+        pos2 = pos.reshape(-1, 2)
+        if not pos2.is_contiguous():
+            pos2 = pos2.contiguous()
+        ctx.npf = npf
+        ctx.save_for_backward(pos2)
+        return K.sine_embed_fwd(pos2, npf, 2 * math.pi).view(*pos.shape[:-1], 2 * npf)
+
+    @staticmethod
+    @K.backward_scope
+    def backward(ctx, g):
+        (pos2,) = ctx.saved_tensors
+        g2 = g.reshape(-1, 2 * ctx.npf)
+        if not g2.is_contiguous():
+            g2 = g2.contiguous()
+        return K.sine_embed_bwd(g2, pos2, ctx.npf, 2 * math.pi).view(*g.shape[:-1], 2), None
+
+
+def sine_embed_ok(pos, d_model):
+    return pos.is_cuda and pos.dtype == torch.float32 and pos.shape[-1] == 2 and d_model % 4 == 0 and d_model >= 4
+
+
+def sine_embed(pos, d_model):
+    return _SineEmbed.apply(pos, d_model)
 
 
 class _TalkingHeadsAttention(Function):
```

Result: slower. 41.61 images/sec (-2.1%).
